# amorim-cleison/sign-language-nlp

Measured on AMD Instinct MI355X. Metric: train seq/s (batch=50,len=48), higher is better.
Workload: dtype bf16x3; 1 GPU; cfg2: Transformer train step E512 H8 N6 F512 batch 50 len 48 |src| 3000 |tgt| 202 dropout 0.1, fwd+CE+bwd+clip(0.5)+SGD(m=.9); launch=eager stream launches (auto: timed both in 9 untimed pre-warmup steps + warmup), per_gpu=independent fit (grid shard)

## Files before the change

### include/slnlp.h

```cpp
#ifndef SLNLP_H
#define SLNLP_H

#include <stdint.h>

#ifdef __cplusplus
extern "C" {
#endif

#define SLNLP_OK 0
#define SLNLP_ERR_INVALID_ARG 1
#define SLNLP_ERR_LAUNCH 2
#define SLNLP_ERR_UNSUPPORTED 3

#define SLNLP_ABI_VERSION 1

const char* slnlp_last_error(void);
int slnlp_abi_version(void);

typedef struct slnlp_gemm_args {
    const float* A; int64_t lda; int32_t a_kmajor;
    const float* B; int64_t ldb; int32_t b_kmajor;
    float* C; int64_t ldc;
    int32_t M, N, K;
    const float* bias;
    int32_t relu;
    const float* gate; int64_t ldg; float gate_scale;
    float drop_p; int32_t drop_site; const unsigned long long* rng;
    const float* resid; int64_t ldr;
    float* rowsum_a;
    int32_t precision;
    int32_t gate_mode;
    const uint16_t* A_hi; const uint16_t* A_lo; int64_t lda_p;
    const uint16_t* B_hi; const uint16_t* B_lo; int64_t ldb_p;
    uint16_t* C_hi; uint16_t* C_lo; int64_t ldc_p;
    int32_t drop_head_dim;
    const float* col_scale;
    uint8_t* C_q8;
    int32_t batch;
    int64_t batch_stride_a, batch_stride_b, batch_stride_c;
} slnlp_gemm_args;

int slnlp_gemm(const slnlp_gemm_args* args, void* stream);
int64_t slnlp_gemm_group_scratch_bytes(const slnlp_gemm_args* jobs, const int32_t* split_k, int njobs);
int slnlp_set_plane_tile(int tile);
int slnlp_set_gemm_ks(int ks);
int slnlp_set_rnn_step_tile(int rows16);
int slnlp_set_fp8_tile(int tile);
int slnlp_gemm_group(const slnlp_gemm_args* jobs, const int32_t* split_k, int njobs, void* scratch,
                     int64_t scratch_bytes, void* stream);
int slnlp_gemm_wd(const slnlp_gemm_args* wgrad, const slnlp_gemm_args* dgrad, void* scratch, int64_t scratch_bytes, void* stream);
int slnlp_gemm_wd_plan(const slnlp_gemm_args* wgrad, const slnlp_gemm_args* dgrad, int32_t* split, int32_t* separate, int32_t* geo_wgrad,
                       int32_t* geo_dgrad);
int slnlp_gemm_rows(const slnlp_gemm_args* args, void* stream);
int slnlp_gemm_rows_bwd(const slnlp_gemm_args* dgrad, const slnlp_gemm_args* wgrad, void* stream);
int slnlp_set_rows_tile(int tile);
int slnlp_quant_rows_fp8(const float* x, int64_t ld, int R, int K, uint8_t* q, int64_t ldq, float* scale, void* stream);
int slnlp_split_planes(const float* x, int64_t ld, int R, int C, uint16_t* hi, uint16_t* lo, int64_t ldp, void* stream);

int slnlp_embed_fwd(const int64_t* ids, int64_t ld_ids, int B, int S, int E, int V,
                    const float* table, const float* pe , float* out,
                    float scale ,
                    float drop_p, int drop_site, const unsigned long long* rng,
                    int64_t nan_idx , void* stream);
int64_t slnlp_embed_bwd_scratch_bytes(int B, int S, int E);
int slnlp_embed_bwd(const int64_t* ids, int64_t ld_ids, int B, int S, int E, int V,
                    const float* dx, float* dtable, float scale,
                    int64_t zero_row ,
                    float drop_p, int drop_site, const unsigned long long* rng,
                    void* scratch, void* stream);

int slnlp_attn_self_fwd(const float* qkv, const int64_t* ids, int64_t ld_ids, int64_t pad_idx,
                        int causal, int B, int S, int H, int dh,
                        float* ctx, float* probs,
                        float drop_p, int drop_site, const unsigned long long* rng, void* stream);
int slnlp_attn_self_bwd(const float* qkv, const float* probs, const float* dctx,
                        int B, int S, int H, int dh, float* dqkv,
                        float drop_p, int drop_site, const unsigned long long* rng, void* stream);

int64_t slnlp_attn_long_scratch_bytes(int B, int S, int H);
int slnlp_attn_self_bwd_long(const float* qkv, const float* probs, const float* dctx, int B, int S, int H, int dh,
                             float* dqkv, float* scratch, float drop_p, int drop_site, const unsigned long long* rng,
                             void* stream);
int slnlp_attn_cross_fwd(const float* q, const float* kv, int64_t ld_kv, int B, int S, int H, int dh,
                         float* ctx, float* probs,
                         float drop_p, int drop_site, const unsigned long long* rng, void* stream);
int slnlp_attn_cross_bwd(const float* q, const float* kv, int64_t ld_kv, const float* probs,
                         const float* dctx, int B, int S, int H, int dh,
                         float* dq, float* dkv, int64_t ld_dkv,
                         float drop_p, int drop_site, const unsigned long long* rng, void* stream);

int slnlp_layernorm_fwd(const float* x, const float* gamma, const float* beta, int rows, int E,
                        float eps, float* y, float* stats, void* stream);
#define SLNLP_LN_MAX_PARTIALS 1024
int slnlp_layernorm_bwd(const float* dy, const float* x, const float* gamma, const float* stats,
                        int rows, int E, const float* add_to_dx, float* dx, float* dx_drop,
                        float drop_p, int drop_site, const unsigned long long* rng,
                        float* partial, int* nblk_out, void* stream);
typedef struct slnlp_ln_reduce_entry {
    const float* partial; float* dgamma; float* dbeta; int32_t nblk; int32_t E;
} slnlp_ln_reduce_entry;
int slnlp_ln_param_reduce(const slnlp_ln_reduce_entry* table_dev, int n, int max_E, void* stream);

int slnlp_lsm_nll(const float* logits, int64_t ld_logits, const int64_t* y, int B, int V,
                  int64_t ignore_index, float* logp, float* loss, float* dlogits, int64_t ld_dlogits,
                  float* row_scratch , void* stream);
int slnlp_lsm_nll_ex(const float* logits, int64_t ld_logits, const int64_t* y, int B, int V, int64_t ignore_index,
                     const float* class_weight, float label_smoothing, int reduction, float* logp, float* loss,
                     float* dlogits, int64_t ld_dlogits, float* row_scratch , void* stream);
int slnlp_lsm_bwd(const float* logp, const float* dlogp, int B, int V, float* dlogits,
                  int64_t ld_dlogits, void* stream);

int slnlp_clip_sgd_step(float* params, const float* grads, float* momentum_buf, int64_t n,
                        const float* lr_dev, float momentum, float max_norm,
                        float* partials , float* norm_out,
                        unsigned long long* rng, void* stream);

int slnlp_clip_sgd_step_ex(float* params, const float* grads, float* momentum_buf, int64_t n, const float* lr_dev,
                           float momentum, float dampening, float weight_decay, int nesterov, float max_norm,
                           float* partials , float* norm_out, float* step_count, int64_t skip_begin,
                           int64_t skip_end, void* stream);
int slnlp_clip_adamw_step(float* params, const float* grads, float* exp_avg, float* exp_avg_sq, int64_t n,
                          const float* lr_dev, float beta1, float beta2, float eps, float weight_decay, float max_norm,
                          float* partials , float* norm_out, float* step_count, int64_t skip_begin,
                          int64_t skip_end, void* stream);

int slnlp_clip_adam_step(float* params, const float* grads, float* exp_avg, float* exp_avg_sq, int64_t n,
                         const float* lr_dev, float beta1, float beta2, float eps, float weight_decay, float max_norm,
                         float* partials , float* norm_out, float* step_count, void* stream);

int slnlp_dropout_mask(float* out, int R, int C, float p, int site,
                       const unsigned long long* rng, void* stream);

typedef struct slnlp_rnn_cell_dir {
    const float* xproj;
    const float* hproj;
    float* h;
    float* c;
    float* hprev_save;
    float* cprev_save;
    float* acts;
    float* hn_save;
    float* out;
    int32_t t, out_row0, out_col0;
} slnlp_rnn_cell_dir;
int slnlp_rnn_cell_fwd(int lstm, const slnlp_rnn_cell_dir* dirs, int ndir, int B, int Hd,
                       const int64_t* lengths, float fill, int64_t ld_out,
                       float drop_p, int drop_site, const unsigned long long* rng, void* stream);
typedef struct slnlp_rnn_step_dir {
    const float* h_in;
    float* h_out;
    const float* w_hh;
    const float* b_hh;
    const float* xproj;
    float* c;
    float* cprev_save;
    float* acts;
    float* hn_save;
    float* out;
    int32_t t, out_row0, out_col0;
} slnlp_rnn_step_dir;
int slnlp_rnn_step_fwd(int lstm, const slnlp_rnn_step_dir* dirs, int ndir, int B, int Hd,
                       const int64_t* lengths, float fill, int64_t ld_out,
                       float drop_p, int drop_site, const unsigned long long* rng, int precision, void* stream);
typedef struct slnlp_rnn_layer_dir {
    float* hprev;
    float* h_final;
    const float* w_hh;
    const float* b_hh;
    const float* xproj;
    float* c;
    float* cprev;
    float* acts;
    float* hn;
    float* out;
    int32_t out_col0;
    int32_t reverse;
} slnlp_rnn_layer_dir;
int slnlp_rnn_layer_fwd(int lstm, const slnlp_rnn_layer_dir* dirs, int ndir, int B, int Hd, int S,
                        const int64_t* lengths, float fill, int64_t ld_out,
                        float drop_p, int drop_site, const unsigned long long* rng, int precision,
                        uint32_t* sync, int* launched, void* stream);
typedef struct slnlp_rnn_cell_bwd_dir {
    float* dh_state; float* dc_state;
    const float* dout;
    const float* acts; const float* cprev_save; const float* hprev_save; const float* hn_save;
    float* dgx; float* dgh; float* carry;
    int32_t t, out_row0, out_col0;
    const float* dh_extra; int64_t extra_stride; int32_t n_extra;
} slnlp_rnn_cell_bwd_dir;
int slnlp_rnn_cell_bwd(int lstm, const slnlp_rnn_cell_bwd_dir* dirs, int ndir, int B, int Hd,
                       const int64_t* lengths, int64_t ld_dout,
                       float drop_p, int drop_site, const unsigned long long* rng, void* stream);

typedef struct slnlp_rnn_step_bwd_dir {
    slnlp_rnn_cell_bwd_dir cell;
    const float* dgh_next;
    const float* w_hh;
} slnlp_rnn_step_bwd_dir;
int slnlp_rnn_step_bwd(int lstm, const slnlp_rnn_step_bwd_dir* dirs, int ndir, int B, int Hd,
                       const int64_t* lengths, int64_t ld_dout,
                       float drop_p, int drop_site, const unsigned long long* rng, int precision, void* stream);

int slnlp_bahdanau_fwd(const float* q, const float* proj_key, const float* value, const float* w_energy,
                       const int64_t* ids, int64_t ld_ids, int64_t pad_idx, int B, int S, int Hd,
                       float* alphas, float* ctx, void* stream);
int slnlp_bahdanau_bwd(const float* q, const float* proj_key, const float* value, const float* w_energy,
// ... 142 lines not shown
```

### sign-language-nlp_amd/csrc/common.hpp

```cpp
#pragma once
#include <vector>
#include <hip/hip_runtime.h>
#include <atomic>
#include <mutex>
#include <stdint.h>
#include <stdio.h>
#include <string.h>

#include "../../include/slnlp.h"

namespace slnlp {

void set_error(const char* fmt, ...);

#define SLNLP_CHECK_ARG(cond, ...)                 \
    do {                                           \
        if (!(cond)) {                             \
            ::slnlp::set_error(__VA_ARGS__);       \
            return SLNLP_ERR_INVALID_ARG;          \
        }                                          \
    } while (0)

#define SLNLP_CHECK_LAUNCH(what)                                              \
    do {                                                                      \
// ... 24 lines not shown
        std::lock_guard<std::mutex> lk(mu);
        if (done[dev].load(std::memory_order_relaxed)) return 0;
        const int rc = init();
        if (rc == 0) done[dev].store(true, std::memory_order_release);
        return rc;
    }
};

#ifndef SLNLP_PROBE_FENCES
#define SLNLP_PROBE_FENCES 0
#endif
__device__ __forceinline__ void probe_kernel_begin() {
#if SLNLP_PROBE_FENCES & 1
    __builtin_amdgcn_fence(__ATOMIC_ACQUIRE, "agent");
    asm volatile("s_waitcnt vmcnt(0)" ::: "memory");
#endif
}
__device__ __forceinline__ void probe_kernel_end() {
#if SLNLP_PROBE_FENCES & 2
    asm volatile("s_waitcnt vmcnt(0)" ::: "memory");
    __builtin_amdgcn_fence(__ATOMIC_RELEASE, "agent");
    asm volatile("s_waitcnt vmcnt(0)" ::: "memory");
#endif
}

struct RngState {
    unsigned long long seed;
    unsigned long long step;
};

struct DropKey { unsigned ks[5]; };
__device__ __forceinline__ DropKey dropout_key(const unsigned long long* rng, int site) {
    const unsigned long long k = rng[0] + 0x9E3779B97F4A7C15ull * rng[1];
    DropKey K;
    K.ks[0] = (unsigned)k; K.ks[1] = (unsigned)(k >> 32); K.ks[2] = (unsigned)site; K.ks[3] = 0u;
    K.ks[4] = 0x1BD11BDAu ^ K.ks[0] ^ K.ks[1] ^ K.ks[2] ^ K.ks[3];
    return K;
}

#ifndef SLNLP_THREEFRY_ROUNDS
#define SLNLP_THREEFRY_ROUNDS 12
#endif
__device__ __forceinline__ uint4 threefry4x32(unsigned c0, unsigned c1, const DropKey& K) {
    constexpr int ROT[8][2] = {{10, 26}, {11, 21}, {13, 27}, {23, 5}, {6, 20}, {17, 11}, {25, 10}, {18, 20}};
    unsigned x0 = c0 + K.ks[0], x1 = c1 + K.ks[1], x2 = K.ks[2], x3 = K.ks[3];
#pragma unroll
    for (int r = 0; r < SLNLP_THREEFRY_ROUNDS; ++r) {
        if ((r & 1) == 0) {
            x0 += x1; x1 = __builtin_rotateleft32(x1, ROT[r & 7][0]) ^ x0;
            x2 += x3; x3 = __builtin_rotateleft32(x3, ROT[r & 7][1]) ^ x2;
        } else {
            x0 += x3; x3 = __builtin_rotateleft32(x3, ROT[r & 7][0]) ^ x0;
            x2 += x1; x1 = __builtin_rotateleft32(x1, ROT[r & 7][1]) ^ x2;
        }
        if ((r & 3) == 3) {
            const int s = (r + 1) >> 2;
            x0 += K.ks[s % 5]; x1 += K.ks[(s + 1) % 5]; x2 += K.ks[(s + 2) % 5]; x3 += K.ks[(s + 3) % 5] + (unsigned)s;
        }
    }
    return make_uint4(x0, x1, x2, x3);
}

__device__ __forceinline__ unsigned drop_cc(unsigned c) { return ((c >> 5) << 4) | (c & 15u); }
__device__ __forceinline__ int drop_half(unsigned c) { return (int)((c >> 4) & 1u); }

__device__ __forceinline__ uint4 dropout_bits8(const DropKey& key, unsigned r4, unsigned cc) { return threefry4x32(cc, r4, key); }

__host__ __device__ __forceinline__ unsigned dropout_threshold(float p) {
    const double t = (double)p * 65536.0 + 0.5;
    return t >= 65535.0 ? 65535u : (unsigned)t;
}

__device__ __forceinline__ unsigned pick_lot(const uint4& v, int half, int r) {
    const unsigned long long lo = (unsigned long long)v.x | ((unsigned long long)v.y << 32);
    const unsigned long long hi = (unsigned long long)v.z | ((unsigned long long)v.w << 32);
    return (unsigned)((half ? hi : lo) >> (16 * (r & 3))) & 0xFFFFu;
}

__device__ __forceinline__ bool dropout_keep(const DropKey& key, unsigned r, unsigned c, unsigned thr) {
    const uint4 b = dropout_bits8(key, r >> 2, drop_cc(c));
    return pick_lot(b, drop_half(c), (int)(r & 3u)) >= thr;
}
__device__ __forceinline__ bool dropout_keep(const unsigned long long* rng, int site,
                                             unsigned r, unsigned c, unsigned thr) {
    return dropout_keep(dropout_key(rng, site), r, c, thr);
}

struct PlaneOut {
    unsigned short* hi = nullptr;
    unsigned short* lo = nullptr;
    unsigned char* q8 = nullptr;
};
__device__ __forceinline__ unsigned pack_fp8x4(float a, float b, float c, float d) {
    a = fminf(fmaxf(a, -448.f), 448.f); b = fminf(fmaxf(b, -448.f), 448.f);
    c = fminf(fmaxf(c, -448.f), 448.f); d = fminf(fmaxf(d, -448.f), 448.f);
    int w = __builtin_amdgcn_cvt_pk_fp8_f32(a, b, 0, false);
    w = __builtin_amdgcn_cvt_pk_fp8_f32(c, d, w, true);
    return (unsigned)w;
}
__device__ __forceinline__ void split_bf16(float x, unsigned short& h, unsigned short& l) {
    const __bf16 hb = (__bf16)x;
    h = __builtin_bit_cast(unsigned short, hb);
    const __bf16 b = (__bf16)(x - (float)hb);
    l = __builtin_bit_cast(unsigned short, b);
}
__device__ __forceinline__ unsigned short head_bf16(float x) { return __builtin_bit_cast(unsigned short, (__bf16)x); }
__device__ __forceinline__ void store_planes1(const PlaneOut& po, long idx, float v) {
    if (!po.hi) return;
    unsigned short h, l;
    split_bf16(v, h, l);
    po.hi[idx] = h;
    po.lo[idx] = l;
    if (po.q8) po.q8[idx] = (unsigned char)(pack_fp8x4(v, 0.f, 0.f, 0.f) & 0xFFu);
}
__device__ __forceinline__ void store_planes4(const PlaneOut& po, long idx, float4 v) {
    if (!po.hi) return;
    unsigned short h[4], l[4];
    split_bf16(v.x, h[0], l[0]); split_bf16(v.y, h[1], l[1]); split_bf16(v.z, h[2], l[2]); split_bf16(v.w, h[3], l[3]);
    uint2 w;
    w.x = h[0] | ((unsigned)h[1] << 16); w.y = h[2] | ((unsigned)h[3] << 16);
    *reinterpret_cast<uint2*>(po.hi + idx) = w;
    w.x = l[0] | ((unsigned)l[1] << 16); w.y = l[2] | ((unsigned)l[3] << 16);
    *reinterpret_cast<uint2*>(po.lo + idx) = w;
    if (po.q8) *reinterpret_cast<unsigned*>(po.q8 + idx) = pack_fp8x4(v.x, v.y, v.z, v.w);
}

template <int CTRL>
__device__ __forceinline__ float dpp_mov(float v) {
    return __builtin_bit_cast(float, __builtin_amdgcn_update_dpp(0, __builtin_bit_cast(int, v), CTRL, 0xF, 0xF, true));
}
constexpr int DPP_XOR1 = 0xB1, DPP_XOR2 = 0x4E;
constexpr int DPP_HALF_MIRROR = 0x141, DPP_MIRROR = 0x140;
__device__ __forceinline__ float lane_bcast(float v, int lane) {
    return __builtin_bit_cast(float, __builtin_amdgcn_readlane(__builtin_bit_cast(int, v), lane));
}
__device__ __forceinline__ float row16_sum(float v) {
    v += dpp_mov<DPP_XOR1>(v);
    v += dpp_mov<DPP_XOR2>(v);
    v += dpp_mov<DPP_HALF_MIRROR>(v);
    v += dpp_mov<DPP_MIRROR>(v);
    return v;
}
__device__ __forceinline__ float row16_max(float v) {
    v = fmaxf(v, dpp_mov<DPP_XOR1>(v));
    v = fmaxf(v, dpp_mov<DPP_XOR2>(v));
    v = fmaxf(v, dpp_mov<DPP_HALF_MIRROR>(v));
    v = fmaxf(v, dpp_mov<DPP_MIRROR>(v));
    return v;
}
__device__ __forceinline__ float wave_sum(float v) {
    v = row16_sum(v);
    return (lane_bcast(v, 0) + lane_bcast(v, 16)) + (lane_bcast(v, 32) + lane_bcast(v, 48));
}
__device__ __forceinline__ float wave_max(float v) {
    v = row16_max(v);
    return fmaxf(fmaxf(lane_bcast(v, 0), lane_bcast(v, 16)), fmaxf(lane_bcast(v, 32), lane_bcast(v, 48)));
}

}

namespace slnlp {
int gemm(const slnlp_gemm_args& a, hipStream_t s);
int gemm_group(const slnlp_gemm_args* jobs, int njobs, hipStream_t s, unsigned wide_mask = 0);
int gemm_planes(const slnlp_gemm_args& a, hipStream_t s);
int gemm_rows(const slnlp_gemm_args& a, hipStream_t s);
int gemm_rows_bwd(const slnlp_gemm_args& dgrad, const slnlp_gemm_args& wgrad, hipStream_t s);
int gemm_planes_init();
int gemm_planes_group(const slnlp_gemm_args* jobs, const int* split_k, int njobs, void* scratch, size_t scratch_bytes,
                      hipStream_t s, bool defer_reduce = false);
size_t gemm_group_scratch_bytes(const slnlp_gemm_args* jobs, const int* split_k, int njobs);
constexpr int WD_MAX_SPLITK = 8;
struct WdPlan { int split, separate; };
WdPlan gemm_planes_wd_plan(const slnlp_gemm_args& wgrad, const slnlp_gemm_args& dgrad);
int gemm_planes_wd(const slnlp_gemm_args& wgrad, const slnlp_gemm_args& dgrad, void* scratch, size_t scratch_bytes, hipStream_t s);
struct QuantRow { long off; int K, pad; };
int quant_rows_fp8(const float* x, int64_t ld, int R, int K, unsigned char* q, int64_t ldq, float* scale, const void* row_table,
                   hipStream_t st);
int split_planes(const float* x, int64_t ld, int R, int C, unsigned short* hi, unsigned short* lo, int64_t ldp, hipStream_t st);
int embed_fwd(const int64_t* ids, int64_t ld_ids, int B, int S, int E, int V, const float* table, const float* pe,
              float* out, float scale, float drop_p, int drop_site, const unsigned long long* rng, int64_t nan_idx,
              hipStream_t st, PlaneOut po = {}, unsigned char* keep_mask = nullptr);
int embed_bwd(const int64_t* ids, int64_t ld_ids, int B, int S, int E, int V, const float* dx, float* dtable,
              float scale, int64_t zero_row, float drop_p, int drop_site, const unsigned long long* rng, void* scratch,
              hipStream_t st, const unsigned char* keep_mask = nullptr);
size_t embed_bwd_scratch_bytes(int B, int S, int E);
int attn_self_fwd(const float* qkv, const int64_t* ids, int64_t ld_ids, int64_t pad_idx, int causal, int B, int S,
                  int H, int dh, float* ctx, float* probs, float drop_p, int drop_site,
                  const unsigned long long* rng, hipStream_t st, PlaneOut po = {});
int attn_self_bwd(const float* qkv, const float* probs, const float* dctx, int B, int S, int H, int dh, float* dqkv,
                  float drop_p, int drop_site, const unsigned long long* rng, hipStream_t st, PlaneOut po = {},
                  float* long_scratch = nullptr);
size_t attn_long_scratch_bytes(int B, int S, int H);
int attn_cross_fwd(const float* q, const float* kv, int64_t ld_kv, int B, int S, int H, int dh, float* ctx,
                   float* probs, float drop_p, int drop_site, const unsigned long long* rng, hipStream_t st);
int attn_cross_bwd(const float* q, const float* kv, int64_t ld_kv, const float* probs, const float* dctx, int B,
                   int S, int H, int dh, float* dq, float* dkv, int64_t ld_dkv, float drop_p, int drop_site,
                   const unsigned long long* rng, hipStream_t st, PlaneOut po = {});
int xmem_fwd(const float* qk, const float* mem, const float* bv, int B, int S, int H, int dh, float* mbar, float* psum, float* probs,
             float* ctx0, float drop_p, int drop_site, const unsigned long long* rng, hipStream_t st);
int xmem_bwd(const float* mem, const float* bv, const float* probs, const float* psum, const float* qk, const float* dmbar,
             const float* dctx, int B, int S, int H, int dh, float* dsc, float* dqk, float* dcp, float* dbv, float* dmem, int accumulate,
             float drop_p, int drop_site, const unsigned long long* rng, hipStream_t st);
int layernorm_fwd(const float* x, const float* gamma, const float* beta, int rows, int E, float eps, float* y,
                  float* stats, hipStream_t st, PlaneOut po = {});
int ln_bwd_blocks(int rows);
bool ln_bwd_fused(int full_rows);
int layernorm_bwd(const float* dy, const float* x, const float* gamma, const float* stats, int rows, int E,
                  const float* add_to_dx, float* dx, float* dx_drop, float drop_p, int drop_site,
                  const unsigned long long* rng, float* partial, int* nblk_out, int full_rows, hipStream_t st,
                  PlaneOut po_dx = {}, PlaneOut po_drop = {});
int attn_init();
int ln_param_reduce(const slnlp_ln_reduce_entry* table_dev, int n, int max_E, hipStream_t st);
struct LnPartialEntry {
    const float* dy;
    const float* x;
    const float* stats;
    float* partial;
    int dec;
    int pad;
};
int ln_param_partial(const LnPartialEntry* table_dev, const LnPartialEntry* single_host, int n, int E, int rows_enc, int rows_dec,
                     int full_rows_enc, int full_rows_dec, hipStream_t st);
int ln_partial_chunk(int rows);
struct LossOpts {
    const float* class_weight = nullptr;
    float label_smoothing = 0.f;
    int reduction = 0;
};
int lsm_nll(const float* logits, int64_t ld_logits, const int64_t* y, int B, int V, int64_t ignore_index, float* logp,
            float* loss, float* dlogits, int64_t ld_dlogits, float* row_scratch, hipStream_t st, hipStream_t loss_st,
            float* logp2 = nullptr, const int* logp2_row = nullptr, float* loss_hist = nullptr, const int* hist_idx = nullptr,
            LossOpts lo = {});
int lsm_bwd(const float* logp, const float* dlogp, int B, int V, float* dlogits, int64_t ld_dlogits, hipStream_t st);
int rnn_cell_fwd(int lstm, const slnlp_rnn_cell_dir* dirs, int ndir, int B, int Hd, const int64_t* lengths, float fill,
                 int64_t ld_out, float drop_p, int drop_site, const unsigned long long* rng, hipStream_t st);
int rnn_step_fwd(int lstm, const slnlp_rnn_step_dir* dirs, int ndir, int B, int Hd, const int64_t* lengths, float fill,
                 int64_t ld_out, float drop_p, int drop_site, const unsigned long long* rng, int precision, hipStream_t st);
int rnn_layer_init();
int rnn_layer_fwd(int lstm, const slnlp_rnn_layer_dir* dirs, int ndir, int B, int Hd, int S, const int64_t* lengths,
                  float fill, int64_t ld_out, float drop_p, int drop_site, const unsigned long long* rng, int precision,
                  unsigned* bar, int* err, int* launched, hipStream_t st);
int rnn_cell_bwd(int lstm, const slnlp_rnn_cell_bwd_dir* dirs, int ndir, int B, int Hd, const int64_t* lengths,
                 int64_t ld_dout, float drop_p, int drop_site, const unsigned long long* rng, hipStream_t st);
bool rnn_step_bwd_covers(int B, int Hd);
int rnn_step_bwd_init();
int rnn_step_bwd(int lstm, const slnlp_rnn_step_bwd_dir* dirs, int ndir, int B, int Hd, const int64_t* lengths, int64_t ld_dout,
                 float drop_p, int drop_site, const unsigned long long* rng, int precision, hipStream_t st);
int bahdanau_fwd(const float* q, const float* pk, const float* val, const float* we, const int64_t* ids,
                 int64_t ld_ids, int64_t pad, int B, int S, int Hd, float* alphas, float* ctx, hipStream_t st);
int bahdanau_bwd(const float* q, const float* pk, const float* val, const float* we, const float* alphas,
                 const float* dctx, int B, int S, int Hd, float* dq, float* dpk, float* dval, float* dwe_part,
                 float* dwe, hipStream_t st);
int add_rows(const float* in, int64_t ld_in, float* out, int64_t ld_out, int R, int C, int accumulate, hipStream_t st);
int tanh_bwd(const float* dy, const float* y, float* out, int64_t n, hipStream_t st);
struct SgdOpts {
    float dampening = 0.f, weight_decay = 0.f;
    int nesterov = 0;
    float* steps = nullptr;
    int64_t skip_begin = 0, skip_end = 0;
};
struct AdamOpts {
    int decoupled = 0;
    int64_t skip_begin = 0, skip_end = 0;
};
int clip_sgd_step(float* params, const float* grads, float* momentum_buf, int64_t n, const float* lr_dev,
                  float momentum, float max_norm, float* partials, float* norm_out, unsigned long long* rng,
                  hipStream_t st, PlaneOut wp = {}, int64_t wp_begin = 0, int64_t wp_end = -1,
                  SgdOpts so = {});
int clip_adam_step(float* params, const float* grads, float* exp_avg, float* exp_avg_sq, int64_t n, const float* lr_dev,
                   float beta1, float beta2, float eps, float weight_decay, float max_norm, float* partials, float* norm_out,
                   unsigned long long* rng, float* step_f, hipStream_t st, PlaneOut wp = {}, int64_t wp_begin = 0, int64_t wp_end = -1,
                   AdamOpts ao = {});
struct TrainOpts {
    float* class_weight = nullptr;
    std::vector<float> class_weight_host;
    float label_smoothing = 0.f;
    int reduction = 0;
    int kind = 0;
    float dampening = 0.f, weight_decay = 0.f;
    int nesterov = 0;
    unsigned gen = 0;
    TrainOpts() = default;
    TrainOpts(const TrainOpts&) = delete;
    TrainOpts& operator=(const TrainOpts&) = delete;
    ~TrainOpts();
    LossOpts loss() const { return LossOpts{class_weight, label_smoothing, reduction}; }
    SgdOpts sgd(float* steps, int64_t skip_begin, int64_t skip_end) const {
        if (kind != 0) return SgdOpts{0.f, 0.f, 0, steps, skip_begin, skip_end};
        return SgdOpts{dampening, weight_decay, nesterov, steps, skip_begin, skip_end};
    }
    AdamOpts adam(int64_t skip_begin, int64_t skip_end) const { return AdamOpts{kind == 2 ? 1 : 0, skip_begin, skip_end}; }
    float adam_weight_decay(float group) const { return kind == 0 ? group : weight_decay; }
    int set_criterion(int V, const float* cw, float eps, int reduction, hipStream_t st, bool* changed);
    int set_update(int kind, float dampening, float weight_decay, int nesterov, bool* changed);
};

unsigned long long params_generation(const float* params);
unsigned long long bump_params_generation(const float* params);
}
```

### sign-language-nlp_amd/csrc/elementwise.hip

```cpp
#include "common.hpp"
#include "launch.hpp"

namespace slnlp {

__device__ __forceinline__ void embed_fwd_body(const long* __restrict__ ids, long ld_ids, int B, int S,
                                                        int E, int V, const float* __restrict__ table,
                                                        const float* __restrict__ pe, float* __restrict__ out,
                                                        float scale, float drop_p, unsigned drop_thr, int drop_site,
                                                        const unsigned long long* __restrict__ rng, long nan_idx,
                                                        PlaneOut po, unsigned char* __restrict__ keep_mask) {
    const int e4 = E >> 2;
    const long total = (long)B * S * e4;
    const float ik = 1.f / (1.f - drop_p);
    for (long idx = blockIdx.x * 256L + threadIdx.x; idx < total; idx += (long)gridDim.x * 256) {
        const int m = (int)(idx / e4), c = (int)(idx % e4) * 4;
        const int s = m / B, b = m % B;
        const long id = ids[(long)b * ld_ids + s];
        float4 v = make_float4(0.f, 0.f, 0.f, 0.f);
        if (id >= 0 && id < V) v = *reinterpret_cast<const float4*>(table + id * E + c);
        const float4 p = pe ? *reinterpret_cast<const float4*>(pe + (long)s * E + c) : make_float4(0.f, 0.f, 0.f, 0.f);
        v.x = v.x * scale + p.x; v.y = v.y * scale + p.y; v.z = v.z * scale + p.z; v.w = v.w * scale + p.w;
        if (drop_p > 0.f) {
            const bool k0 = dropout_keep(rng, drop_site, m, c + 0, drop_thr), k1 = dropout_keep(rng, drop_site, m, c + 1, drop_thr);
            const bool k2 = dropout_keep(rng, drop_site, m, c + 2, drop_thr), k3 = dropout_keep(rng, drop_site, m, c + 3, drop_thr);
// ... 108 lines not shown
        if ((tid & 63) == 0) match[tid >> 6] = bal;
        __syncthreads();
        if (tid == 0) {
            int n = nlist;
            for (int w = 0; w < 4; ++w) {
                unsigned long long bits = match[w];
                while (bits && n < 1024) {
                    list[n++] = base + w * 64 + __ffsll((long long)bits) - 1;
                    bits &= bits - 1;
                }
            }
            nlist = n;
        }
        __syncthreads();
    }
    const int n = nlist;
    __shared__ __attribute__((aligned(16))) float red[4][256];
    const int wave = tid >> 6, lane = tid & 63, per = (n + 3) / 4;
    const int i0 = wave * per, i1 = (i0 + per < n) ? i0 + per : n;
    for (int c0 = 0; c0 < E; c0 += 256) {
        const int c = c0 + lane * 4;
        float4 acc = make_float4(0.f, 0.f, 0.f, 0.f);
        if (c < E) {
            for (int i = i0; i < i1; i += 4) {
                float4 g[4];
#pragma unroll
                for (int u = 0; u < 4; ++u)
                    g[u] = (i + u < i1) ? *reinterpret_cast<const float4*>(partial + (long)list[i + u] * E + c)
                                        : make_float4(0.f, 0.f, 0.f, 0.f);
#pragma unroll
                for (int u = 0; u < 4; ++u) { acc.x += g[u].x; acc.y += g[u].y; acc.z += g[u].z; acc.w += g[u].w; }
            }
        }
        if (c0 > 0) __syncthreads();
        *reinterpret_cast<float4*>(&red[wave][lane * 4]) = acc;
        __syncthreads();
        if (wave == 0 && c < E) {
            float4 r = *reinterpret_cast<const float4*>(&red[0][lane * 4]);
#pragma unroll
            for (int w = 1; w < 4; ++w) {
                const float4 q = *reinterpret_cast<const float4*>(&red[w][lane * 4]);
                r.x += q.x; r.y += q.y; r.z += q.z; r.w += q.w;
            }
            r.x *= scale; r.y *= scale; r.z *= scale; r.w *= scale;
            *reinterpret_cast<float4*>(dtable + (long)id * E + c) = r;
        }
    }
}
SLNLP_ZKERNEL(embed_bwd_combine_kernel, 256, embed_bwd_combine_body)

__device__ __forceinline__ void embed_bwd_small_body(const long* __restrict__ ids, long ld_ids, int B, int S, int E, int V,
                                                     const float* __restrict__ dx, float* __restrict__ dtable, float scale,
                                                     float drop_p, unsigned drop_thr, int drop_site,
                                                     const unsigned long long* __restrict__ rng) {
    const int M = B * S, lane = threadIdx.x & 63, m = blockIdx.x;
    int my_id = -1;
    if (lane < M) {
        const long v = ids[(long)(lane % B) * ld_ids + (lane / B)];
        my_id = (v < 0 || v >= V) ? -1 : (int)v;
    }
    if (m < V && __ballot(my_id == m) == 0ull) {
        for (int c = threadIdx.x * 4; c < E; c += 1024) *reinterpret_cast<float4*>(dtable + (long)m * E + c) = make_float4(0.f, 0.f, 0.f, 0.f);
    }
    if (m >= M) return;
    const float ik = 1.f / (1.f - drop_p);
    const int id = __builtin_amdgcn_readlane(my_id, __builtin_amdgcn_readfirstlane(m));
    const unsigned long long mask = __ballot(my_id == id && id >= 0);
    const bool first = id >= 0 && (mask & ((1ull << m) - 1ull)) == 0ull;
    if (!first) return;
    __shared__ __attribute__((aligned(16))) float red[4][256];
    const int wave = threadIdx.x >> 6;
    const unsigned long long wmask = mask & (0xFFFFull << (16 * wave));
    for (int c0 = 0; c0 < E; c0 += 256) {
        const int c = c0 + lane * 4;
        float4 acc = make_float4(0.f, 0.f, 0.f, 0.f);
        if (c < E) {
            unsigned long long bits = wmask;
            while (bits) {
                int k[4];
#pragma unroll
                for (int u = 0; u < 4; ++u) {
                    k[u] = bits ? __ffsll((long long)bits) - 1 : -1;
                    bits &= bits - 1;
                }
                float4 g[4];
#pragma unroll
                for (int u = 0; u < 4; ++u)
                    g[u] = k[u] >= 0 ? load_dx_row(dx, k[u], E, c, drop_p, ik, drop_thr, drop_site, rng, nullptr)
                                     : make_float4(0.f, 0.f, 0.f, 0.f);
#pragma unroll
                for (int u = 0; u < 4; ++u) { acc.x += g[u].x; acc.y += g[u].y; acc.z += g[u].z; acc.w += g[u].w; }
            }
        }
        if (c0 > 0) __syncthreads();
        *reinterpret_cast<float4*>(&red[wave][lane * 4]) = acc;
        __syncthreads();
        if (wave == 0 && c < E) {
            float4 r = *reinterpret_cast<const float4*>(&red[0][lane * 4]);
#pragma unroll
            for (int w = 1; w < 4; ++w) {
                const float4 q = *reinterpret_cast<const float4*>(&red[w][lane * 4]);
                r.x += q.x; r.y += q.y; r.z += q.z; r.w += q.w;
            }
            r.x *= scale; r.y *= scale; r.z *= scale; r.w *= scale;
            *reinterpret_cast<float4*>(dtable + (long)id * E + c) = r;
        }
    }
}
SLNLP_ZKERNEL(embed_bwd_small_kernel, 256, embed_bwd_small_body)

int embed_fwd(const int64_t* ids, int64_t ld_ids, int B, int S, int E, int V, const float* table, const float* pe,
              float* out, float scale, float drop_p, int drop_site, const unsigned long long* rng, int64_t nan_idx,
              hipStream_t st, PlaneOut po, unsigned char* keep_mask) {
    SLNLP_CHECK_ARG(ids && table && out, "embed_fwd: null pointer");
    SLNLP_CHECK_ARG(B > 0 && S > 0 && V > 0 && E > 0 && E % 4 == 0, "embed_fwd: bad shape B=%d S=%d E=%d V=%d", B, S, E, V);
    SLNLP_CHECK_ARG(drop_p >= 0.f && drop_p < 1.f && (drop_p == 0.f || rng), "embed_fwd: bad dropout args");
    const long total = (long)B * S * (E / 4);
    int grid = ceil_div(total, 256);
    if (grid > 2048) grid = 2048;
    SLNLP_TRY(zlaunch(embed_fwd_kernel, dim3(grid), 256, 0, st, "embed_fwd",
                      (const long*)ids, (long)ld_ids, B, S, E, V, table, pe, out, scale, drop_p, dropout_threshold(drop_p), drop_site, rng, (long)nan_idx, po, keep_mask));
    return 0;
}

size_t embed_bwd_scratch_bytes(int B, int S, int E) {
    return ((size_t)B * S * E * sizeof(float) + (size_t)B * S * sizeof(int) + 255) & ~(size_t)255;
}

int embed_bwd(const int64_t* ids, int64_t ld_ids, int B, int S, int E, int V, const float* dx, float* dtable,
              float scale, int64_t zero_row, float drop_p, int drop_site, const unsigned long long* rng, void* scratch,
              hipStream_t st, const unsigned char* keep_mask) {
    SLNLP_CHECK_ARG(ids && dx && dtable && scratch, "embed_bwd: null pointer");
    SLNLP_CHECK_ARG(B > 0 && S > 0 && V > 0 && E > 0 && E % 4 == 0, "embed_bwd: bad shape");
    SLNLP_CHECK_ARG((long)B * S <= 65536, "embed_bwd: more than 65536 tokens per batch");
    SLNLP_CHECK_ARG(drop_p >= 0.f && drop_p < 1.f && (drop_p == 0.f || rng), "embed_bwd: bad dropout args");
    const int M = B * S;
    if (M <= EMB_CHUNK && !keep_mask) {
        SLNLP_TRY(zlaunch(embed_bwd_small_kernel, dim3(M > V ? M : V), 256, 0, st, "embed_bwd_small",
                          (const long*)ids, (long)ld_ids, B, S, E, V, dx, dtable, scale, drop_p, dropout_threshold(drop_p), drop_site, rng));
        if (zero_row >= 0 && zero_row < V) SLNLP_TRY(fill_zero(dtable + zero_row * E, (size_t)E * sizeof(float), st));
        return 0;
    }
    SLNLP_TRY(fill_zero(dtable, (size_t)V * E * sizeof(float), st));
    float* partial = (float*)scratch;
    int* pid = (int*)(partial + (size_t)M * E);
    SLNLP_TRY(zlaunch(embed_bwd_chunk_kernel, dim3(M), 256, 0, st, "embed_bwd_chunk",
                      (const long*)ids, (long)ld_ids, B, S, E, V, dx, partial, pid, drop_p, dropout_threshold(drop_p), drop_site, rng, keep_mask));
    SLNLP_TRY(zlaunch(embed_bwd_combine_kernel, dim3(M), 256, 0, st, "embed_bwd_combine",
                      pid, M, E, partial, dtable, scale));
    if (zero_row >= 0 && zero_row < V) SLNLP_TRY(fill_zero(dtable + zero_row * E, (size_t)E * sizeof(float), st));
    return 0;
}

constexpr int LN_MAXU = 4;

__device__ __forceinline__ void layernorm_fwd_body(const float* __restrict__ x,
                                                            const float* __restrict__ gamma,
                                                            const float* __restrict__ beta, int rows, int E,
                                                            float eps, float* __restrict__ y,
                                                            float* __restrict__ stats, PlaneOut po) {
    const int lane = threadIdx.x & 63, wave = threadIdx.x >> 6;
    const int row = blockIdx.x * 4 + wave;
    if (row >= rows) return;
    const float* xr = x + (long)row * E;
    float4 v[LN_MAXU], g[LN_MAXU], bt[LN_MAXU];
#pragma unroll
    for (int u = 0; u < LN_MAXU; ++u) {
        const int c = lane * 4 + u * 256;
        const bool in = c < E;
        v[u] = in ? *reinterpret_cast<const float4*>(xr + c) : make_float4(0.f, 0.f, 0.f, 0.f);
        g[u] = in ? *reinterpret_cast<const float4*>(gamma + c) : make_float4(0.f, 0.f, 0.f, 0.f);
        bt[u] = in ? *reinterpret_cast<const float4*>(beta + c) : make_float4(0.f, 0.f, 0.f, 0.f);
    }
    float s = 0.f;
#pragma unroll
    for (int u = 0; u < LN_MAXU; ++u) s += v[u].x + v[u].y + v[u].z + v[u].w;
    const float mean = wave_sum(s) / (float)E;
    float q = 0.f;
#pragma unroll
    for (int u = 0; u < LN_MAXU; ++u) {
        if (lane * 4 + u * 256 < E) {
            const float a = v[u].x - mean, b = v[u].y - mean, cc = v[u].z - mean, d = v[u].w - mean;
            q += a * a + b * b + cc * cc + d * d;
        }
    }
    const float rstd = 1.f / sqrtf(wave_sum(q) / (float)E + eps);
#pragma unroll
    for (int u = 0; u < LN_MAXU; ++u) {
        const int c = lane * 4 + u * 256;
        if (c < E) {
            float4 o;
            o.x = (v[u].x - mean) * rstd * g[u].x + bt[u].x; o.y = (v[u].y - mean) * rstd * g[u].y + bt[u].y;
            o.z = (v[u].z - mean) * rstd * g[u].z + bt[u].z; o.w = (v[u].w - mean) * rstd * g[u].w + bt[u].w;
            *reinterpret_cast<float4*>(y + (long)row * E + c) = o;
            store_planes4(po, (long)row * E + c, o);
        }
    }
    if (lane == 0 && stats) {
        stats[2 * row] = mean;
        stats[2 * row + 1] = rstd;
    }
}
SLNLP_ZKERNEL(layernorm_fwd_kernel, 256, layernorm_fwd_body)

template <int U, int GS, int RB, bool FUSE>
__device__ __forceinline__ void layernorm_bwd_rows(
    const float* __restrict__ dy, const float* __restrict__ x, const float* __restrict__ gamma,
    const float* __restrict__ stats, int rows, int E, const float* __restrict__ add_to_dx, float* __restrict__ dx,
    float* __restrict__ dx_drop, float drop_p, unsigned drop_thr, int drop_site,
    const unsigned long long* __restrict__ rng, PlaneOut po_dx, PlaneOut po_drop, float* __restrict__ partial, int chunk_rows, int nchunks) {
    const int lane = threadIdx.x & 63, wave = threadIdx.x >> 6;
    const float invE = 1.f / (float)E, ik = 1.f / (1.f - drop_p);
    const bool want_drop = dx_drop != nullptr || po_drop.hi != nullptr;
    const bool drop = want_drop && drop_p > 0.f;
    const int unit = FUSE ? (int)blockIdx.x : blockIdx.x * (int)(blockDim.x >> 6) + wave;
    float4 ag[U], ab[U];
#pragma unroll
    for (int u = 0; u < U; ++u) ag[u] = ab[u] = make_float4(0.f, 0.f, 0.f, 0.f);
    const int row_begin = FUSE ? unit * chunk_rows + wave * GS : unit * GS;
    const int row_end = FUSE ? ((unit + 1) * chunk_rows < rows ? (unit + 1) * chunk_rows : rows) : row_begin + GS;
    const int row_step = FUSE ? 4 * GS : GS;
    if (!FUSE && row_begin >= rows) return;
    DropKey dkey = {};
    if (drop) dkey = dropout_key(rng, drop_site);
    float4 g[U];
#pragma unroll
    for (int u = 0; u < U; ++u)
        if (lane * 4 + u * 256 < E) g[u] = *reinterpret_cast<const float4*>(gamma + lane * 4 + u * 256);
#pragma unroll 1
    for (int row0 = row_begin; row0 < row_end; row0 += row_step)
#pragma unroll
    for (int i0 = 0; i0 < GS; i0 += RB) {
        float4 d[RB][U], v[RB][U];
        float mean[RB], rstd[RB], s1[RB], s2[RB];
#pragma unroll
        for (int i = 0; i < RB; ++i) {
            const int row = row0 + i0 + i < rows ? row0 + i0 + i : rows - 1;
            mean[i] = stats[2 * row];
            rstd[i] = stats[2 * row + 1];
#pragma unroll
            for (int u = 0; u < U; ++u) {
                const int c = lane * 4 + u * 256;
                if (c < E) {
                    d[i][u] = *reinterpret_cast<const float4*>(dy + (long)row * E + c);
                    v[i][u] = *reinterpret_cast<const float4*>(x + (long)row * E + c);
                }
            }
        }
#pragma unroll
        for (int i = 0; i < RB; ++i) {
            float a1 = 0.f, a2 = 0.f;
#pragma unroll
            for (int u = 0; u < U; ++u) {
                if (lane * 4 + u * 256 < E) {
                    const float4 dd = d[i][u], vv = v[i][u];
                    const float4 xh = make_float4((vv.x - mean[i]) * rstd[i], (vv.y - mean[i]) * rstd[i], (vv.z - mean[i]) * rstd[i], (vv.w - mean[i]) * rstd[i]);
                    const float4 gv = make_float4(dd.x * g[u].x, dd.y * g[u].y, dd.z * g[u].z, dd.w * g[u].w);
                    a1 += gv.x + gv.y + gv.z + gv.w;
                    a2 += gv.x * xh.x + gv.y * xh.y + gv.z * xh.z + gv.w * xh.w;
                }
            }
            s1[i] = wave_sum(a1) * invE;
            s2[i] = wave_sum(a2) * invE;
        }
#pragma unroll
        for (int u = 0; u < U; ++u) {
            const int c = lane * 4 + u * 256;
            if (c >= E) continue;
            uint4 kb[4];
            const int half = drop_half((unsigned)c);
            if (drop) {
#pragma unroll
                for (int e = 0; e < 4; ++e) kb[e] = dropout_bits8(dkey, (unsigned)(row0 + i0) >> 2, drop_cc((unsigned)(c + e)));
            }
#pragma unroll
            for (int i = 0; i < RB; ++i) {
                const int row = row0 + i0 + i;
                if (row >= rows) continue;
                const int wsel = row & 3;
                const float4 dd = d[i][u], vv = v[i][u];
                const float4 xh = make_float4((vv.x - mean[i]) * rstd[i], (vv.y - mean[i]) * rstd[i], (vv.z - mean[i]) * rstd[i], (vv.w - mean[i]) * rstd[i]);
                const float4 gv = make_float4(dd.x * g[u].x, dd.y * g[u].y, dd.z * g[u].z, dd.w * g[u].w);
                if (FUSE) {
                    ag[u].x += dd.x * xh.x; ag[u].y += dd.y * xh.y; ag[u].z += dd.z * xh.z; ag[u].w += dd.w * xh.w;
                    ab[u].x += dd.x; ab[u].y += dd.y; ab[u].z += dd.z; ab[u].w += dd.w;
                }
                float4 o;
                o.x = rstd[i] * (gv.x - s1[i] - xh.x * s2[i]); o.y = rstd[i] * (gv.y - s1[i] - xh.y * s2[i]);
                o.z = rstd[i] * (gv.z - s1[i] - xh.z * s2[i]); o.w = rstd[i] * (gv.w - s1[i] - xh.w * s2[i]);
                if (add_to_dx) {
                    const float4 a = *reinterpret_cast<const float4*>(add_to_dx + (long)row * E + c);
                    o.x += a.x; o.y += a.y; o.z += a.z; o.w += a.w;
                }
                *reinterpret_cast<float4*>(dx + (long)row * E + c) = o;
                store_planes4(po_dx, (long)row * E + c, o);
                if (want_drop) {
                    if (drop) {
                        o.x = pick_lot(kb[0], half, wsel) >= drop_thr ? o.x * ik : 0.f;
                        o.y = pick_lot(kb[1], half, wsel) >= drop_thr ? o.y * ik : 0.f;
                        o.z = pick_lot(kb[2], half, wsel) >= drop_thr ? o.z * ik : 0.f;
                        o.w = pick_lot(kb[3], half, wsel) >= drop_thr ? o.w * ik : 0.f;
                    }
                    if (dx_drop) *reinterpret_cast<float4*>(dx_drop + (long)row * E + c) = o;
                    store_planes4(po_drop, (long)row * E + c, o);
                }
            }
        }
    }
    if (FUSE) {
        __shared__ float4 red[4][2][U * 64];
#pragma unroll
        for (int u = 0; u < U; ++u) {
            red[wave][0][u * 64 + lane] = ag[u];
            red[wave][1][u * 64 + lane] = ab[u];
        }
        __syncthreads();
        for (int q = threadIdx.x; q < 2 * U * 64; q += 256) {
            const int which = q / (U * 64), slot = q - which * (U * 64), c = (slot & 63) * 4 + (slot >> 6) * 256;
            if (c >= E) continue;
            float4 t = red[0][which][slot];
#pragma unroll
            for (int k = 1; k < 4; ++k) {
                const float4 o = red[k][which][slot];
                t.x += o.x; t.y += o.y; t.z += o.z; t.w += o.w;
            }
            *reinterpret_cast<float4*>(partial + ((long)unit * 2 + which) * E + c) = t;
        }
    }
}

#define SLNLP_LN_BWD_BODY(name, U, GS, RB, FUSE)                                                                                    \
    __device__ __forceinline__ void name(const float* __restrict__ dy, const float* __restrict__ x, const float* __restrict__ gamma, \
                                         const float* __restrict__ stats, int rows, int E, const float* __restrict__ add_to_dx,     \
                                         float* __restrict__ dx, float* __restrict__ dx_drop, float drop_p, unsigned drop_thr,       \
                                         int drop_site, const unsigned long long* __restrict__ rng, PlaneOut po_dx,                  \
                                         PlaneOut po_drop, float* __restrict__ partial, int chunk_rows, int nchunks) {               \
        layernorm_bwd_rows<U, GS, RB, FUSE>(dy, x, gamma, stats, rows, E, add_to_dx, dx, dx_drop, drop_p, drop_thr, drop_site, rng, \
                                            po_dx, po_drop, partial, chunk_rows, nchunks);                                          \
    }
SLNLP_LN_BWD_BODY(layernorm_bwd_body_u1g4, 1, 4, 4, false)
SLNLP_LN_BWD_BODY(layernorm_bwd_body_u2g4, 2, 4, 4, false)
SLNLP_LN_BWD_BODY(layernorm_bwd_body_u4g4, 4, 4, 2, false)
SLNLP_LN_BWD_BODY(layernorm_bwd_body_u1g1, 1, 1, 1, false)
SLNLP_LN_BWD_BODY(layernorm_bwd_body_u2g1, 2, 1, 1, false)
SLNLP_LN_BWD_BODY(layernorm_bwd_body_u4g1, 4, 1, 1, false)
SLNLP_LN_BWD_BODY(layernorm_bwd_body_u1g4f, 1, 4, 4, true)
SLNLP_LN_BWD_BODY(layernorm_bwd_body_u2g4f, 2, 4, 4, true)
SLNLP_LN_BWD_BODY(layernorm_bwd_body_u4g4f, 4, 4, 2, true)
// ... 662 lines not shown
```

### sign-language-nlp_amd/csrc/gemm_rows.hip

```cpp
#include <algorithm>
#include <atomic>

#include "common.hpp"
#include "gemm_jobs.hpp"
#include "launch.hpp"

namespace slnlp {

typedef __attribute__((ext_vector_type(8))) __bf16 bf16x8;
typedef __attribute__((ext_vector_type(4))) float f32x4;

struct RowsParams {
    slnlp_gemm_args a;
    unsigned drop_thr;
    float drop_scale;
};
__device__ __forceinline__ RowsParams as_global(RowsParams p) {
    launder(p.a);
    return p;
}

#if SLNLP_PROBE_FENCES == 256
constexpr int RTS_MAX = 1 << 14, RTS_W = 6;
__device__ unsigned long long g_rts[RTS_MAX][RTS_W];
__device__ unsigned g_rts_n;
#define RTS_MARK(slot) do { if (threadIdx.x == 0) rts[slot] = __builtin_amdgcn_s_memrealtime(); } while (0)
#else
#define RTS_MARK(slot) do { } while (0)
#endif

constexpr int RT_THREADS = 512, RT_WAVES = 8;
constexpr int RT_MAX_KTILES = 16;

typedef __attribute__((ext_vector_type(4))) short s16x4;
typedef __attribute__((ext_vector_type(8))) short s16x8;
typedef __attribute__((address_space(3))) void* lds_vp;
typedef __attribute__((address_space(1))) const void* glb_vp;

constexpr int RT_IMG = 64 * 16;
__device__ __forceinline__ void rows_dma_image(const unsigned short* __restrict__ plane, long ld, int k0, int r0, unsigned short* img, int lane) {
#pragma unroll
    for (int q = 0; q < 2; ++q) {
        const unsigned short* src = plane + (long)(k0 + 32 * q + (lane >> 1)) * ld + r0 + 8 * (lane & 1);
        __builtin_amdgcn_global_load_lds((glb_vp)src, (lds_vp)(img + q * 512), 16, 0, 0);
    }
}
__device__ __forceinline__ bf16x8 rows_tr_frag(const unsigned short* img, int kk, int lane) {
    const int i = lane & 15, kb = kk * 32 + ((lane >> 4) << 3) + (i >> 2);
    const unsigned short* p0 = img + kb * 16 + ((i & 3) << 2);
    typedef __attribute__((address_space(3))) s16x4* lds_p;
    const s16x4 v0 = __builtin_amdgcn_ds_read_tr16_b64_v4i16((lds_p)(p0));
    const s16x4 v1 = __builtin_amdgcn_ds_read_tr16_b64_v4i16((lds_p)(p0 + 4 * 16));
    const s16x8 v = {v0[0], v0[1], v0[2], v0[3], v1[0], v1[1], v1[2], v1[3]};
    return __builtin_bit_cast(bf16x8, v);
}

template <int NSPLIT>
__device__ __forceinline__ void rows_split8(const float (&x)[8], bf16x8& hi, bf16x8& lo) {
#pragma unroll
    for (int e = 0; e < 8; ++e) {
        const __bf16 h = (__bf16)x[e];
        hi[e] = h;
        if (NSPLIT == 3) lo[e] = (__bf16)(x[e] - (float)h);
    }
}
__device__ __forceinline__ void rows_load8(const float* __restrict__ p, float (&x)[8]) {
    const float4 a = *reinterpret_cast<const float4*>(p), b = *reinterpret_cast<const float4*>(p + 4);
    x[0] = a.x; x[1] = a.y; x[2] = a.z; x[3] = a.w; x[4] = b.x; x[5] = b.y; x[6] = b.z; x[7] = b.w;
}
constexpr int RT_FIMG = 64 * 16;
__device__ __forceinline__ void rows_dma_image_f32(const float* __restrict__ W, long ld, int k0, int c0, int N, float* img, int lane) {
#pragma unroll
    for (int q = 0; q < 4; ++q) {
        const int c = min(c0 + 4 * (lane & 3), N - 4);
        const float* src = W + (long)(k0 + 16 * q + (lane >> 2)) * ld + c;
        __builtin_amdgcn_global_load_lds((glb_vp)src, (lds_vp)(img + q * 256), 16, 0, 0);
    }
}
__device__ __forceinline__ void rows_img_col8(const float* img, int kk, int lane, float (&x)[8]) {
    const float* p = img + (kk * 32 + ((lane >> 4) << 3)) * 16 + (lane & 15);
#pragma unroll
    for (int e = 0; e < 8; ++e) x[e] = p[e * 16];
}

template <int NSPLIT, int MT, int NT, bool BK>
__device__ __forceinline__ void rows_tile(const RowsParams& p, int bx, int by, float* part) {
    static_assert(MT * NT <= RT_WAVES, "one epilogue tile per wave");
    const slnlp_gemm_args& g = p.a;
    const int tid = threadIdx.x, lane = tid & 63, wave = __builtin_amdgcn_readfirstlane(tid >> 6);
#if SLNLP_PROBE_FENCES == 256
    unsigned long long rts[RTS_W] = {0, 0, 0, 0, 0, 0};
    struct RtsFlush {
        unsigned long long* t;
        __device__ ~RtsFlush() {
            if (threadIdx.x == 0) {
                t[4] = __builtin_amdgcn_s_memrealtime();
                t[5] = ((unsigned long long)(gridDim.x * gridDim.y) << 32) | (unsigned)(blockIdx.y * gridDim.x + blockIdx.x);
                const unsigned i = atomicAdd(&g_rts_n, 1u) & (unsigned)(RTS_MAX - 1);
                for (int k = 0; k < RTS_W; ++k) g_rts[i][k] = t[k];
            }
        }
    } rts_flush{rts};
    RTS_MARK(0);
#endif
    const int bn0 = bx * 16 * NT, bm0 = by * 16 * MT;
    const int M = g.M, N = g.N;
    const int ktiles = (g.K + 63) >> 6;
    const int am_last = ((M + 15) / 16 - 1) * 16, bn_last = ((N + 15) / 16 - 1) * 16;
    const long koct = 8 * (lane >> 4);
    const unsigned short *ah[MT], *al[MT];
    const float* bw[NT];
    int bcol[NT];
#pragma unroll
    for (int i = 0; i < MT; ++i) {
        const long off = (long)(min(bm0 + 16 * i, am_last) + (lane & 15)) * g.lda_p + koct;
        ah[i] = g.A_hi + off; al[i] = g.A_lo + off;
    }
#pragma unroll
    for (int j = 0; j < NT; ++j) {
        bcol[j] = min(bn0 + 16 * j, bn_last);
        bw[j] = g.B + (long)min(bcol[j] + (lane & 15), N - 1) * g.ldb + koct;
    }
    float* bimg = part + (size_t)ktiles * MT * NT * 256 + wave * NT * RT_FIMG;

    const int ei = wave / NT, ej = wave % NT;
    const int gm0 = bm0 + 16 * ei + ((lane >> 4) << 2), gn = bn0 + 16 * ej + (lane & 15);
    const bool live = wave < MT * NT && gn < N && gm0 < M;
    float bias = 0.f, gt[4] = {0.f, 0.f, 0.f, 0.f}, rs[4] = {0.f, 0.f, 0.f, 0.f};
    DropKey dkey = {};
    auto epilogue_loads = [&]() {
        if (!live) return;
        if (g.bias) bias = g.bias[gn];
#pragma unroll
        for (int r = 0; r < 4; ++r) {
            const int gm = gm0 + r < M ? gm0 + r : gm0;
            if (g.gate) gt[r] = g.gate[(long)gm * g.ldg + gn];
            if (g.resid) rs[r] = g.resid[(long)gm * g.ldr + gn];
        }
        if (g.drop_p > 0.f) dkey = dropout_key(g.rng, g.drop_site);
    };

    for (int t = wave; t < ktiles; t += RT_WAVES) {
        bf16x8 fa[2][MT], la[2][MT], fb[2][NT], lb[2][NT];
        if (!BK) {
            if (t != wave) asm volatile("s_waitcnt lgkmcnt(0)" ::: "memory");
#pragma unroll
            for (int j = 0; j < NT; ++j) rows_dma_image_f32(g.B, g.ldb, t * 64, bcol[j], N, bimg + j * RT_FIMG, lane);
        }
#pragma unroll
        for (int kk = 0; kk < 2; ++kk) {
            const int k = t * 64 + kk * 32;
            if (BK) {
#pragma unroll
                for (int j = 0; j < NT; ++j) {
                    float x[8];
                    rows_load8(bw[j] + k, x);
                    rows_split8<NSPLIT>(x, fb[kk][j], lb[kk][j]);
                }
            }
#pragma unroll
            for (int i = 0; i < MT; ++i) {
                fa[kk][i] = *reinterpret_cast<const bf16x8*>(ah[i] + k);
                if (NSPLIT == 3) la[kk][i] = *reinterpret_cast<const bf16x8*>(al[i] + k);
            }
        }
        if (t == wave) epilogue_loads();
        if (!BK) {
            asm volatile("s_waitcnt vmcnt(0)" ::: "memory");
#pragma unroll
            for (int kk = 0; kk < 2; ++kk)
#pragma unroll
                for (int j = 0; j < NT; ++j) {
                    float x[8];
                    rows_img_col8(bimg + j * RT_FIMG, kk, lane, x);
                    rows_split8<NSPLIT>(x, fb[kk][j], lb[kk][j]);
                }
        }
#if SLNLP_PROBE_FENCES == 256
        if (t == 0) { asm volatile("s_waitcnt vmcnt(0)" ::: "memory"); RTS_MARK(1); }
#endif
        f32x4 acc[MT][NT];
#pragma unroll
        for (int i = 0; i < MT; ++i)
#pragma unroll
            for (int j = 0; j < NT; ++j) acc[i][j] = f32x4{0.f, 0.f, 0.f, 0.f};
#pragma unroll
        for (int kk = 0; kk < 2; ++kk)
#pragma unroll
            for (int i = 0; i < MT; ++i)
#pragma unroll
                for (int j = 0; j < NT; ++j) {
                    if (NSPLIT == 3) {
                        acc[i][j] = __builtin_amdgcn_mfma_f32_16x16x32_bf16(la[kk][i], fb[kk][j], acc[i][j], 0, 0, 0);
                        acc[i][j] = __builtin_amdgcn_mfma_f32_16x16x32_bf16(fa[kk][i], lb[kk][j], acc[i][j], 0, 0, 0);
                    }
                    acc[i][j] = __builtin_amdgcn_mfma_f32_16x16x32_bf16(fa[kk][i], fb[kk][j], acc[i][j], 0, 0, 0);
                }
#pragma unroll
        for (int i = 0; i < MT; ++i)
#pragma unroll
            for (int j = 0; j < NT; ++j) *reinterpret_cast<f32x4*>(part + (((t * MT + i) * NT + j) * 64 + lane) * 4) = acc[i][j];
    }
    if (wave >= ktiles) epilogue_loads();
    RTS_MARK(2);
    __syncthreads();
    if (wave >= MT * NT) return;
    f32x4 acc = *reinterpret_cast<const f32x4*>(part + (wave * 64 + lane) * 4);
    for (int t = 1; t < ktiles; ++t) acc += *reinterpret_cast<const f32x4*>(part + ((t * MT * NT + wave) * 64 + lane) * 4);
    RTS_MARK(3);
    if (!live) return;

    unsigned lot[4] = {0u, 0u, 0u, 0u};
    if (g.drop_p > 0.f) {
        if (g.drop_head_dim == 0) {
            const uint4 bits = dropout_bits8(dkey, (unsigned)gm0 >> 2, drop_cc((unsigned)gn));
            const int h = drop_half((unsigned)gn);
#pragma unroll
            for (int r = 0; r < 4; ++r) lot[r] = pick_lot(bits, h, r);
        } else {
#pragma unroll
            for (int r = 0; r < 4; ++r) {
                const unsigned rh = (unsigned)(gm0 + r) * (unsigned)(N / g.drop_head_dim) + (unsigned)(gn / g.drop_head_dim);
                lot[r] = pick_lot(dropout_bits8(dkey, rh >> 2, 0u), 0, (int)(rh & 3u));
            }
        }
    }
#pragma unroll
    for (int r = 0; r < 4; ++r) {
        const int gm = gm0 + r;
        if (gm >= M) break;
        float v = acc[r] + bias;
        if (g.relu == 1) v = fmaxf(v, 0.f);
        else if (g.relu == 2) v = tanhf(v);
        if (g.gate) v = g.gate_mode == 1 ? v * (1.f - gt[r] * gt[r]) : (gt[r] > 0.f ? v * g.gate_scale : 0.f);
        if (g.drop_p > 0.f) v = (lot[r] >= p.drop_thr) ? v * p.drop_scale : 0.f;
        if (g.resid) v += rs[r];
        if (g.C) g.C[(long)gm * g.ldc + gn] = v;
        if (g.C_hi) {
            unsigned short h, l;
            split_bf16(v, h, l);
            g.C_hi[(long)gm * g.ldc_p + gn] = h;
            if (g.C_lo) g.C_lo[(long)gm * g.ldc_p + gn] = l;
        }
    }
}

template <int NSPLIT, int WM>
__device__ __forceinline__ void rows_wgrad_unit(const slnlp_gemm_args& g, int unit, unsigned short* smem) {
    constexpr int NP = NSPLIT == 3 ? 2 : 1;
    const int tid = threadIdx.x, lane = tid & 63, wave = __builtin_amdgcn_readfirstlane(tid >> 6);
    const int M = g.M, N = g.N, ktiles = (g.K + 63) >> 6;
    const int units_n = (N + 127) / 128, um = unit / units_n, un = unit - um * units_n;
    const int m0 = um * 16 * WM, n0 = un * 128 + wave * 16, m_last = ((M + 15) / 16 - 1) * 16;
    const bool active = n0 < N;
    unsigned short* aimg = smem;
    unsigned short* bimg = smem + WM * 2 * RT_IMG + wave * 2 * RT_IMG;
    f32x4 total[WM], rsum[WM];
#pragma unroll
    for (int i = 0; i < WM; ++i) { total[i] = f32x4{0.f, 0.f, 0.f, 0.f}; rsum[i] = f32x4{0.f, 0.f, 0.f, 0.f}; }
    const bool do_rs = g.rowsum_a != nullptr && un == 0 && wave == 0;
    bf16x8 ones;
#pragma unroll
    for (int e = 0; e < 8; ++e) ones[e] = (__bf16)1.0f;
#if SLNLP_PROBE_FENCES == 256
    unsigned long long rts[RTS_W] = {0, 0, 0, 0, 0, 0};
    struct RtsFlushW {
        unsigned long long* t;
        unsigned tag;
        __device__ ~RtsFlushW() {
            if (threadIdx.x == 0) {
                t[4] = __builtin_amdgcn_s_memrealtime();
                t[5] = ((unsigned long long)(gridDim.x * gridDim.y) << 32) | tag | (unsigned)(blockIdx.y * gridDim.x + blockIdx.x);
                const unsigned i = atomicAdd(&g_rts_n, 1u) & (unsigned)(RTS_MAX - 1);
                for (int k = 0; k < RTS_W; ++k) g_rts[i][k] = t[k];
            }
        }
    } rts_flush{rts, 0x80000000u | (g.rowsum_a != nullptr && un == 0 ? 0x40000000u : 0u)};
    RTS_MARK(0);
#endif
    for (int t = 0; t < ktiles; ++t) {
        if (t) {
            asm volatile("s_waitcnt lgkmcnt(0)" ::: "memory");
            __syncthreads();
        }
        for (int im = wave; im < WM * NP; im += RT_WAVES) {
            const int i = im / NP, pl = im - i * NP;
            rows_dma_image(pl ? g.A_lo : g.A_hi, g.lda_p, t * 64, min(m0 + 16 * i, m_last), aimg + (2 * i + pl) * RT_IMG, lane);
        }
        if (active) {
            rows_dma_image(g.B_hi, g.ldb_p, t * 64, n0, bimg, lane);
            if (NSPLIT == 3) rows_dma_image(g.B_lo, g.ldb_p, t * 64, n0, bimg + RT_IMG, lane);
        }
        asm volatile("s_waitcnt vmcnt(0)" ::: "memory");
        __syncthreads();
#if SLNLP_PROBE_FENCES == 256
        if (t == 0) RTS_MARK(1);
#endif
        if (active) {
            bf16x8 fb[2], lb[2];
#pragma unroll
            for (int kk = 0; kk < 2; ++kk) {
                fb[kk] = rows_tr_frag(bimg, kk, lane);
                if (NSPLIT == 3) lb[kk] = rows_tr_frag(bimg + RT_IMG, kk, lane);
            }
#pragma unroll
            for (int i = 0; i < WM; ++i) {
                f32x4 acc = f32x4{0.f, 0.f, 0.f, 0.f}, rs = f32x4{0.f, 0.f, 0.f, 0.f};
#pragma unroll
                for (int kk = 0; kk < 2; ++kk) {
                    const bf16x8 fa = rows_tr_frag(aimg + (2 * i) * RT_IMG, kk, lane);
                    if (NSPLIT == 3) {
                        const bf16x8 la = rows_tr_frag(aimg + (2 * i + 1) * RT_IMG, kk, lane);
                        acc = __builtin_amdgcn_mfma_f32_16x16x32_bf16(la, fb[kk], acc, 0, 0, 0);
                        acc = __builtin_amdgcn_mfma_f32_16x16x32_bf16(fa, lb[kk], acc, 0, 0, 0);
                        if (do_rs) rs = __builtin_amdgcn_mfma_f32_16x16x32_bf16(la, ones, rs, 0, 0, 0);
                    }
                    acc = __builtin_amdgcn_mfma_f32_16x16x32_bf16(fa, fb[kk], acc, 0, 0, 0);
                    if (do_rs) rs = __builtin_amdgcn_mfma_f32_16x16x32_bf16(fa, ones, rs, 0, 0, 0);
                }
                total[i] = t == 0 ? acc : total[i] + acc;
                if (do_rs) rsum[i] = t == 0 ? rs : rsum[i] + rs;
            }
        }
#if SLNLP_PROBE_FENCES == 256
        if (t == 0) RTS_MARK(2);
#endif
    }
    RTS_MARK(3);
    if (!active) return;
    const int gn = n0 + (lane & 15);
#pragma unroll
    for (int i = 0; i < WM; ++i) {
        const int gm0 = m0 + 16 * i + ((lane >> 4) << 2);
        if (gn < N) {
#pragma unroll
            for (int r = 0; r < 4; ++r)
                if (gm0 + r < M) g.C[(long)(gm0 + r) * g.ldc + gn] = total[i][r];
        }
        if (do_rs && (lane & 15) == 0) {
#pragma unroll
            for (int r = 0; r < 4; ++r)
                if (gm0 + r < M) g.rowsum_a[gm0 + r] = rsum[i][r];
        }
    }
}

template <int NSPLIT, int MT, int NT>
__device__ __forceinline__ void gemm_rows_body(RowsParams p) {
    extern __shared__ __attribute__((aligned(16))) float part[];
    rows_tile<NSPLIT, MT, NT, true>(p, blockIdx.x, blockIdx.y, part);
}

struct RowsBwdParams {
    RowsParams d;
    slnlp_gemm_args w;
};
__device__ __forceinline__ RowsBwdParams as_global(RowsBwdParams p) {
    launder(p.d.a);
    launder(p.w);
    return p;
}
template <int NSPLIT, int MT, int NT>
__device__ __forceinline__ void gemm_rows_bwd_body(RowsBwdParams p) {
    extern __shared__ __attribute__((aligned(16))) float part[];
    const int gx = (p.d.a.N + 16 * NT - 1) / (16 * NT), gy = (p.d.a.M + 16 * MT - 1) / (16 * MT), nd = gx * gy;
    const int id = blockIdx.x;
    if (id < nd) rows_tile<NSPLIT, MT, NT, false>(p.d, id % gx, id / gx, part);
    else rows_wgrad_unit<NSPLIT, MT>(p.w, id - nd, reinterpret_cast<unsigned short*>(part));
}

struct RowsGeo { int mt, nt; };
constexpr int RT_NGEO = 3;
constexpr RowsGeo RT_GEO[RT_NGEO] = {{1, 1}, {4, 1}, {4, 2}};
#define SLNLP_ROWS_KERNEL(NS, G)                                                                                          \
    __device__ __forceinline__ void gemm_rows_body_##NS##_##G(RowsParams p) { gemm_rows_body<NS, RT_GEO[G].mt, RT_GEO[G].nt>(p); } \
    SLNLP_ZKERNEL(gemm_rows_kernel_##NS##_##G, RT_THREADS, gemm_rows_body_##NS##_##G)                                     \
    __device__ __forceinline__ void gemm_rows_bwd_body_##NS##_##G(RowsBwdParams p) { gemm_rows_bwd_body<NS, RT_GEO[G].mt, RT_GEO[G].nt>(p); } \
    SLNLP_ZKERNEL(gemm_rows_bwd_kernel_##NS##_##G, RT_THREADS, gemm_rows_bwd_body_##NS##_##G)
SLNLP_ROWS_KERNEL(3, 0)
SLNLP_ROWS_KERNEL(3, 1)
SLNLP_ROWS_KERNEL(3, 2)
SLNLP_ROWS_KERNEL(1, 0)
SLNLP_ROWS_KERNEL(1, 1)
SLNLP_ROWS_KERNEL(1, 2)

using RowsKernel = void (*)(Pack<RowsParams>, const Pack<RowsParams>*);
using RowsBwdKernel = void (*)(Pack<RowsBwdParams>, const Pack<RowsBwdParams>*);
static RowsKernel rows_kernel(int precision, int geo) {
    if (precision == 3) return geo == 0 ? gemm_rows_kernel_3_0 : geo == 1 ? gemm_rows_kernel_3_1 : gemm_rows_kernel_3_2;
    return geo == 0 ? gemm_rows_kernel_1_0 : geo == 1 ? gemm_rows_kernel_1_1 : gemm_rows_kernel_1_2;
}
static RowsBwdKernel rows_bwd_kernel(int precision, int geo) {
    if (precision == 3) return geo == 0 ? gemm_rows_bwd_kernel_3_0 : geo == 1 ? gemm_rows_bwd_kernel_3_1 : gemm_rows_bwd_kernel_3_2;
    return geo == 0 ? gemm_rows_bwd_kernel_1_0 : geo == 1 ? gemm_rows_bwd_kernel_1_1 : gemm_rows_bwd_kernel_1_2;
}
static size_t rows_lds(int geo, int K) { return (size_t)ceil_div(K, 64) * RT_GEO[geo].mt * RT_GEO[geo].nt * 64 * 4 * sizeof(float); }
static size_t rows_bwd_lds(int geo, int K) {
    const size_t d = rows_lds(geo, K) + (size_t)RT_WAVES * RT_GEO[geo].nt * RT_FIMG * sizeof(float);
    const size_t w = (size_t)(RT_GEO[geo].mt + RT_WAVES) * 2 * RT_IMG * sizeof(unsigned short);
    return d > w ? d : w;
}
static dim3 rows_grid(int geo, int M, int N) { return dim3(ceil_div(N, 16 * RT_GEO[geo].nt), ceil_div(M, 16 * RT_GEO[geo].mt)); }
static int rows_wgrad_units(const slnlp_gemm_args& w, int geo) { return ceil_div(w.M, 16 * RT_GEO[geo].mt) * ceil_div(w.N, 128); }

static std::atomic<int> g_rows_geo{[] { const char* e = getenv("SLNLP_ROWS_TILE"); const int v = e ? atoi(e) : -1; return v >= 0 && v < RT_NGEO ? v : -1; }()};
constexpr size_t RT_LDS_MAX = 160 * 1024;
static int rows_geo(int M, int N, int K, int fits, bool bwd) {
    const int forced = g_rows_geo.load(std::memory_order_relaxed);
    auto fits_lds = [&](int geo) { return (bwd ? rows_bwd_lds(geo, K) : rows_lds(geo, K)) <= RT_LDS_MAX; };
    if (forced >= 0 && fits_lds(forced)) return forced;
    int best = 0;
    long best_cost = -1;
    for (int geo = 0; geo < RT_NGEO; ++geo) {
        if (!fits_lds(geo)) continue;
        const dim3 gr = rows_grid(geo, M, N);
        const long wunits = bwd ? (long)ceil_div(K, 16 * RT_GEO[geo].mt) * ceil_div(N, 128) : 0;
        const long units = ((long)gr.x * gr.y + wunits) * fits, rounds = (units + 255) / 256;
        const long cost = rounds * (16L * (RT_GEO[geo].mt + RT_GEO[geo].nt) * K * 4 + 16384);
        if (best_cost < 0 || cost < best_cost) { best_cost = cost; best = geo; }
    }
    return best;
}

static int rows_init() {
    static DeviceOnce once;
    return once.run([]() -> int {
        bool ok = true;
        for (int prec = 1; prec <= 3; prec += 2)
            for (int geo = 0; geo < RT_NGEO; ++geo)
                ok = ok && hipFuncSetAttribute((const void*)rows_kernel(prec, geo), hipFuncAttributeMaxDynamicSharedMemorySize,
                                               (int)std::min(rows_lds(geo, 64 * RT_MAX_KTILES), RT_LDS_MAX)) == hipSuccess &&
                     hipFuncSetAttribute((const void*)rows_bwd_kernel(prec, geo), hipFuncAttributeMaxDynamicSharedMemorySize,
                                         (int)std::min(rows_bwd_lds(geo, 64 * RT_MAX_KTILES), RT_LDS_MAX)) == hipSuccess;
        if (!ok) {
            set_error("gemm_rows: cannot raise dynamic LDS limit: %s", hipGetErrorString(hipGetLastError()));
            return SLNLP_ERR_LAUNCH;
        }
        return 0;
    });
}

const void* gemm_rows_for_fits(const void* fn, const void* recorded_args, int fits, dim3* grid, size_t* lds) {
    int prec = 0;
    bool bwd = false;
    for (int geo = 0; geo < RT_NGEO; ++geo) {
        if (fn == (const void*)rows_kernel(3, geo)) prec = 3;
        if (fn == (const void*)rows_kernel(1, geo)) prec = 1;
        if (fn == (const void*)rows_bwd_kernel(3, geo)) { prec = 3; bwd = true; }
        if (fn == (const void*)rows_bwd_kernel(1, geo)) { prec = 1; bwd = true; }
    }
    if (!prec) return nullptr;
    if (bwd) {
        const RowsBwdParams& P = *reinterpret_cast<const RowsBwdParams*>(recorded_args);
        const int geo = rows_geo(P.d.a.M, P.d.a.N, P.d.a.K, fits, true);
        const dim3 gr = rows_grid(geo, P.d.a.M, P.d.a.N);
        *grid = dim3(gr.x * gr.y + rows_wgrad_units(P.w, geo));
        *lds = rows_bwd_lds(geo, P.d.a.K);
        return (const void*)rows_bwd_kernel(prec, geo);
    }
    const slnlp_gemm_args& a = reinterpret_cast<const RowsParams*>(recorded_args)->a;
    const int geo = rows_geo(a.M, a.N, a.K, fits, false);
    *grid = rows_grid(geo, a.M, a.N);
    *lds = rows_lds(geo, a.K);
    return (const void*)rows_kernel(prec, geo);
}

static int check_rows_job(const slnlp_gemm_args& a, bool b_kmajor, const char* who) {
    SLNLP_CHECK_ARG(a.A_hi && a.B, "%s: A as bf16 planes (A_hi / A_lo / lda_p) and the weight B as fp32 (B / ldb) required", who);
    SLNLP_CHECK_ARG(a.a_kmajor && (a.b_kmajor != 0) == b_kmajor, "%s: operand layouts (A k-major; B k-major for a forward product, m-major for a data gradient)", who);
    SLNLP_CHECK_ARG(a.C || a.C_hi, "%s: no output", who);
    SLNLP_CHECK_ARG(a.M > 0 && a.N > 0 && a.K > 0, "%s: bad shape M=%d N=%d K=%d", who, a.M, a.N, a.K);
    SLNLP_CHECK_ARG(a.precision == 1 || (a.precision == 3 && a.A_lo), "%s: precision 1, or 3 with A's lo plane", who);
    SLNLP_CHECK_ARG(a.lda_p % 64 == 0 && a.lda_p >= a.K, "%s: A's plane row stride must be a multiple of 64 and cover K (zero-padded)", who);
    SLNLP_CHECK_ARG(a.K % 64 == 0 && a.ldb % 4 == 0 && a.ldb >= (b_kmajor ? a.K : a.N) && (b_kmajor || a.N % 4 == 0),
                    "%s: K must be a multiple of 64 (the fp32 weight has no padding), ldb a multiple of 4 that covers a row", who);
    SLNLP_CHECK_ARG((((uintptr_t)a.A_hi | (uintptr_t)a.A_lo | (uintptr_t)a.B) & 15) == 0, "%s: operands must be 16-byte aligned", who);
    SLNLP_CHECK_ARG(!a.C || a.ldc >= a.N, "%s: ldc < N", who);
    SLNLP_CHECK_ARG(!a.C_hi || a.ldc_p >= a.N, "%s: ldc_p < N", who);
    SLNLP_CHECK_ARG(a.drop_p >= 0.f && a.drop_p < 1.f && (a.drop_p == 0.f || a.rng), "%s: bad dropout args", who);
    SLNLP_CHECK_ARG(!a.gate || a.ldg >= a.N, "%s: ldg too small", who);
    SLNLP_CHECK_ARG(!a.resid || a.ldr >= a.N, "%s: ldr too small", who);
    SLNLP_CHECK_ARG(!a.rowsum_a && a.batch <= 1, "%s: no row sums, no batched jobs", who);
    SLNLP_CHECK_ARG(a.drop_head_dim >= 0 && (a.drop_head_dim == 0 || a.N % a.drop_head_dim == 0), "%s: drop_head_dim %d does not divide N %d", who,
                    a.drop_head_dim, a.N);
    SLNLP_CHECK_ARG(ceil_div(a.K, 64) <= RT_MAX_KTILES, "%s: K = %d > %d (the workgroup's partial tiles live in LDS)", who, a.K, 64 * RT_MAX_KTILES);
    return 0;
}

int gemm_rows_bwd(const slnlp_gemm_args& dgrad, const slnlp_gemm_args& wgrad, hipStream_t st) {
    SLNLP_TRY(check_rows_job(dgrad, false, "gemm_rows_bwd (dgrad)"));
    const slnlp_gemm_args& w = wgrad;
    SLNLP_CHECK_ARG(w.A_hi && w.B_hi && w.C && !w.a_kmajor && !w.b_kmajor, "gemm_rows_bwd (wgrad): m-major operand planes and an fp32 output required");
    SLNLP_CHECK_ARG(w.precision == dgrad.precision && (w.precision == 1 || (w.A_lo && w.B_lo)), "gemm_rows_bwd (wgrad): same precision as the dgrad, lo planes for 3");
    SLNLP_CHECK_ARG(w.M > 0 && w.N > 0 && w.K > 0 && w.lda_p % 64 == 0 && w.ldb_p % 64 == 0 && w.lda_p >= w.M && w.ldb_p >= w.N && w.ldc >= w.N,
                    "gemm_rows_bwd (wgrad): bad shape / strides");
    SLNLP_CHECK_ARG((((uintptr_t)w.A_hi | (uintptr_t)w.B_hi | (uintptr_t)w.A_lo | (uintptr_t)w.B_lo) & 15) == 0, "gemm_rows_bwd (wgrad): planes must be 16-byte aligned");
    SLNLP_CHECK_ARG(!w.bias && !w.gate && !w.resid && w.drop_p == 0.f && !w.C_hi && w.relu == 0 && w.batch <= 1, "gemm_rows_bwd (wgrad): no epilogue");
    RowsBwdParams p;
    p.d.a = dgrad;
    p.d.drop_thr = dropout_threshold(dgrad.drop_p);
    p.d.drop_scale = 1.f / (1.f - dgrad.drop_p);
    p.w = wgrad;
    SLNLP_TRY(rows_init());
    const int geo = rows_geo(dgrad.M, dgrad.N, dgrad.K, 1, true);
    const dim3 gr = rows_grid(geo, dgrad.M, dgrad.N);
    return zlaunch(rows_bwd_kernel(dgrad.precision, geo), dim3(gr.x * gr.y + rows_wgrad_units(wgrad, geo)), RT_THREADS, rows_bwd_lds(geo, dgrad.K), st,
                   "gemm_rows_bwd", p);
}

int gemm_rows(const slnlp_gemm_args& a, hipStream_t st) {
    SLNLP_TRY(check_rows_job(a, true, "gemm_rows"));
    RowsParams p;
    p.a = a;
    p.drop_thr = dropout_threshold(a.drop_p);
    p.drop_scale = 1.f / (1.f - a.drop_p);
    SLNLP_TRY(rows_init());
    const int geo = rows_geo(a.M, a.N, a.K, 1, false);
    return zlaunch(rows_kernel(a.precision, geo), rows_grid(geo, a.M, a.N), RT_THREADS, rows_lds(geo, a.K), st, "gemm_rows", p);
}

}

#if SLNLP_PROBE_FENCES == 256
extern "C" int slnlp_probe_rows_ts(unsigned long long* dst, int max_entries) {
    unsigned n = 0;
    if (hipDeviceSynchronize() != hipSuccess) return -1;
    if (hipMemcpyFromSymbol(&n, HIP_SYMBOL(slnlp::g_rts_n), sizeof(n)) != hipSuccess) return -1;
    if (n > (unsigned)slnlp::RTS_MAX) n = slnlp::RTS_MAX;
    if ((int)n > max_entries) n = max_entries;
    if (n && hipMemcpyFromSymbol(dst, HIP_SYMBOL(slnlp::g_rts), (size_t)n * slnlp::RTS_W * sizeof(unsigned long long)) != hipSuccess) return -1;
    const unsigned zero = 0;
    if (hipMemcpyToSymbol(HIP_SYMBOL(slnlp::g_rts_n), &zero, sizeof(zero)) != hipSuccess) return -1;
    return (int)n;
}
#endif

extern "C" int slnlp_gemm_rows_bwd(const slnlp_gemm_args* dgrad, const slnlp_gemm_args* wgrad, void* stream) {
    if (!dgrad || !wgrad) {
        slnlp::set_error("gemm_rows_bwd: null args");
        return SLNLP_ERR_INVALID_ARG;
    }
    return slnlp::gemm_rows_bwd(*dgrad, *wgrad, (hipStream_t)stream);
}

extern "C" int slnlp_set_rows_tile(int tile) {
    if (tile < -1 || tile >= slnlp::RT_NGEO) {
        slnlp::set_error("set_rows_tile: %d (-1 = automatic, 0 = 16 x 16, 1 = 64 x 16, 2 = 64 x 32 outputs per workgroup)", tile);
        return SLNLP_ERR_INVALID_ARG;
    }
    slnlp::g_rows_geo.store(tile, std::memory_order_relaxed);
    return 0;
}

extern "C" int slnlp_gemm_rows(const slnlp_gemm_args* args, void* stream) {
    if (!args) {
        slnlp::set_error("gemm_rows: null args");
        return SLNLP_ERR_INVALID_ARG;
    }
    return slnlp::gemm_rows(*args, (hipStream_t)stream);
}
```

### sign-language-nlp_amd/csrc/tf_plan.hip

```cpp
#include <map>
#include <string>
#include <vector>

#include "common.hpp"
#include "launch.hpp"
#include "tf_plan.hpp"

using namespace slnlp;

extern "C" {

int slnlp_tf_num_params(const slnlp_tf_config* cfg) {
    if (check_cfg(cfg)) return -1;
    return (int)build_layout(*cfg).ents.size();
}

int slnlp_tf_param_info(const slnlp_tf_config* cfg, int i, char* name, int64_t shape[2], int* ndim, int64_t* offset) {
    SLNLP_TRY(check_cfg(cfg));
    Layout L = build_layout(*cfg);
    SLNLP_CHECK_ARG(i >= 0 && i < (int)L.ents.size(), "tf_param_info: index %d out of range", i);
    const ParamEnt& e = L.ents[i];
    if (name) {
        strncpy(name, e.name.c_str(), 127);
        name[127] = 0;
    }
    if (shape) {
        shape[0] = e.shape[0];
        shape[1] = e.shape[1];
    }
    if (ndim) *ndim = e.ndim;
    if (offset) *offset = e.off;
    return 0;
}

int64_t slnlp_tf_arena_floats(const slnlp_tf_config* cfg) {
    if (check_cfg(cfg)) return -1;
    return build_layout(*cfg).total;
}

int64_t slnlp_tf_workspace_bytes(const slnlp_tf_config* cfg) {
    if (check_cfg(cfg)) return -1;
    return (int64_t)carve(*cfg, nullptr).bytes;
}

void slnlp_tf_destroy(slnlp_tf_plan* plan) {
    if (!plan) return;
    if (!plan->graphs.empty()) (void)hipDeviceSynchronize();
    else destroy_sync(plan->destroy_sync);
    for (auto& kv : plan->graphs) (void)hipGraphExecDestroy(kv.second);
    delete plan;
}

int slnlp_tf_create(const slnlp_tf_config* cfg, const slnlp_tf_buffers* buf, slnlp_tf_plan** out) {
    SLNLP_TRY(check_cfg(cfg));
    SLNLP_CHECK_ARG(buf && out, "tf_create: null argument");
    SLNLP_CHECK_ARG(buf->params && buf->grads && buf->momentum && buf->pe && buf->workspace && buf->rng && buf->lr &&
                        buf->scalars,
                    "tf_create: every buffer pointer is required");
    SLNLP_CHECK_ARG((((uintptr_t)buf->params | (uintptr_t)buf->grads | (uintptr_t)buf->momentum |
                      (uintptr_t)buf->workspace | (uintptr_t)buf->pe) & 255) == 0,
                    "tf_create: arenas / workspace / pe must be 256-byte aligned");
    slnlp_tf_plan* p = new slnlp_tf_plan();
    p->cfg = *cfg;
    p->buf = *buf;
    p->L = build_layout(*cfg);
    p->w = carve(*cfg, buf->workspace);
    bool ok = attn_init() == 0 && gemm_planes_init() == 0;
    p->use_planes = (cfg->E % 64 == 0) && (cfg->F % 64 == 0);
    p->wgrad_np = wgrad_passes();
    p->dgrad_np = dgrad_passes();
    {
        const char* e = getenv("SLNLP_DEC_ROWS");
        p->use_rows = p->use_planes && cfg->E <= 1024 && cfg->F <= 1024 && !(e && atoi(e) == 0);
    }
    if (ok && cfg->precision == 8) {
        std::vector<QuantRow> rows;
        auto block = [&](long off, int nrows, int K) {
            p->qrow0[off] = (long)rows.size();
            for (int r = 0; r < nrows; ++r) rows.push_back(QuantRow{off + (long)r * K, K, 0});
        };
        const int E = cfg->E, F = cfg->F;
        for (int i = 0; i < cfg->N; ++i) {
            const EncP& q = p->L.enc[i];
            block(q.in_w, 3 * E, E); block(q.out_w, E, E); block(q.l1_w, F, E); block(q.l2_w, E, F);
        }
        ok = (long)rows.size() == p->w.n_qrows &&
             hipMemcpy(p->w.qrow_table, rows.data(), rows.size() * sizeof(QuantRow), hipMemcpyHostToDevice) == hipSuccess;
    }
    std::vector<slnlp_ln_reduce_entry> tab;
    std::vector<LnPartialEntry> ptab;
    const int nbE = p->nbE = ln_bwd_blocks(cfg->B * cfg->S), nbD = p->nbD = ln_bwd_blocks(cfg->B);
    auto ent = [&](float* part, long gw, long gb, int dec, const float* dy, const float* x, const float* stats) {
        slnlp_ln_reduce_entry e;
        e.partial = part; e.dgamma = p->G(gw); e.dbeta = p->G(gb); e.nblk = dec ? nbD : nbE; e.E = cfg->E;
        tab.push_back(e);
        LnPartialEntry q;
        q.dy = dy; q.x = x; q.stats = stats; q.partial = part; q.dec = dec; q.pad = 0;
        ptab.push_back(q);
    };
    {
        const Ws& w = p->w;
        const int N = cfg->N;
        for (int i = 0; i < N; ++i) {
            const EncA& a = w.enc[i];
            ent(a.lnp1, p->L.enc[i].n1_w, p->L.enc[i].n1_b, 0, a.gx1, a.y1, a.st1);
            ent(a.lnp2, p->L.enc[i].n2_w, p->L.enc[i].n2_b, 0, i + 1 < N ? w.enc[i + 1].gx0 : w.gxl, a.y2, a.st2);
        }
        ent(w.lnp_mem, p->L.encn_w, p->L.encn_b, 0, w.gmem, w.enc[N - 1].x2, w.st_mem);
        for (int i = 0; i < N; ++i) {
            const DecA& a = w.dec[i];
            ent(a.lnp1, p->L.dec[i].n1_w, p->L.dec[i].n1_b, 1, a.gt1, a.y1, a.st1);
            ent(a.lnp2, p->L.dec[i].n2_w, p->L.dec[i].n2_b, 1, a.gt2, a.y2, a.st2);
            ent(a.lnp3, p->L.dec[i].n3_w, p->L.dec[i].n3_b, 1, i + 1 < N ? w.dec[i + 1].gt0 : w.gtl, a.y3, a.st3);
        }
        ent(w.lnp_fin, p->L.decn_w, p->L.decn_b, 1, w.gfin, w.dec[N - 1].t3, w.st_fin);
    }
    ok = ok && hipMemcpy(p->w.ln_table, tab.data(), tab.size() * sizeof(tab[0]), hipMemcpyHostToDevice) == hipSuccess &&
         hipMemcpy(p->w.ln_ptable, ptab.data(), ptab.size() * sizeof(ptab[0]), hipMemcpyHostToDevice) == hipSuccess &&
         hipMemset(buf->grads, 0, p->L.total * sizeof(float)) == hipSuccess &&
         hipStreamSynchronize(nullptr) == hipSuccess;
    if (!ok) {
        set_error("tf_create: device initialisation failed: %s", hipGetErrorString(hipGetLastError()));
        slnlp_tf_destroy(p);
        return SLNLP_ERR_LAUNCH;
    }
    *out = p;
    return 0;
}

}

int slnlp_tf_plan::dec_self_block(int l, const float* t, const PP* tp, int B, float p, hipStream_t st) const {
    const slnlp_tf_plan* pl = this;
    const int E = cfg.E, dh = E / cfg.H;
    const DecP& q = L.dec[l];
    const DecA& a = w.dec[l];
    if (use_rows) {
        SLNLP_TRY(pl->linear_r(*tp, B, E, q.sin_w + 2L * E * E, E, pl->P(q.sin_b) + 2 * E, a.v, E, 0, p, pl->dec_site(l, 0), nullptr, &a.vp, st, dh));
        SLNLP_TRY(pl->linear_r(a.vp, B, E, q.sout_w, E, pl->P(q.sout_b), a.y1, E, 0, p, pl->dec_site(l, 1), t, nullptr, st));
        SLNLP_TRY(layernorm_fwd(a.y1, pl->P(q.n1_w), pl->P(q.n1_b), B, E, 1e-5f, a.t1, a.st1, st, a.t1p.out()));
        SLNLP_TRY(pl->linear_r(a.t1p, B, E, q.cin_w, E, pl->P(q.cin_b), a.q, E, 0, 0.f, 0, nullptr, nullptr, st));
        return 0;
    }
    SLNLP_TRY(pl->linear(t, B, E, pl->P(q.sin_w) + 2L * E * E, E, pl->P(q.sin_b) + 2 * E, a.v, E, 0, p, pl->dec_site(l, 0), nullptr, st, dh));
    SLNLP_TRY(pl->linear(a.v, B, E, pl->P(q.sout_w), E, pl->P(q.sout_b), a.y1, E, 0, p, pl->dec_site(l, 1), t, st));
    SLNLP_TRY(layernorm_fwd(a.y1, pl->P(q.n1_w), pl->P(q.n1_b), B, E, 1e-5f, a.t1, a.st1, st));
    SLNLP_TRY(pl->linear(a.t1, B, E, pl->P(q.cin_w), E, pl->P(q.cin_b), a.q, E, 0, 0.f, 0, nullptr, st));
    return 0;
}

int slnlp_tf_plan::forward_impl(const int64_t* X, const int64_t* y, int B, int train, float* logp_out, hipStream_t st) {
    slnlp_tf_plan* pl = this;
    const slnlp_tf_config& c = pl->cfg;
    const int E = c.E, F = c.F, H = c.H, S = c.S, dh = E / H, M = S * B, Vp = (int)align_up(c.Vt, 4);
    const float p = train ? c.dropout : 0.f;
    const unsigned long long* rng = pl->buf.rng;
    pl->last_B = B; pl->last_p = p; pl->last_X = X; pl->last_y = y;

    const bool up = use_planes;
    if (up) {
        SLNLP_TRY(prepare_planes(B, st));
        SLNLP_TRY(ensure_wplanes(st));
        SLNLP_TRY(ensure_wq(st));
    }
    SLNLP_TRY(embed_fwd(y, 1, B, 1, E, c.Vt, pl->P(L.tgt_emb), pl->buf.pe, w.t0, sqrtf((float)E), p, SITE_TGT_EMB, rng, c.pad_tgt, st,
                        use_rows ? w.t0p.out() : PlaneOut{}));
    SLNLP_TRY(dec_self_block(0, w.t0, &w.t0p, B, p, st));
    SLNLP_TRY(embed_fwd(X, S, B, S, E, c.Vs, pl->P(L.src_emb), pl->buf.pe, w.x0, sqrtf((float)E), p, SITE_SRC_EMB, rng, -1, st,
                        up ? w.x0p.out() : PlaneOut{}, w.emb_keep));

    const float* x = w.x0;
    const PP* xp = &w.x0p;
    for (int l = 0; l < c.N; ++l) {
        const EncP& q = L.enc[l];
        const EncA& a = w.enc[l];
        if (up) {
            SLNLP_TRY(pl->linear_p(*xp, M, E, q.in_w, 3 * E, pl->P(q.in_b), a.qkv, 3 * E, 0, 0.f, 0, nullptr, nullptr, st));
            SLNLP_TRY(attn_self_fwd(a.qkv, X, S, c.pad_src, 1, B, S, H, dh, S <= 64 ? nullptr : a.ctx, a.probs, p, pl->enc_site(l, 0), rng, st, a.ctxp.out()));
            SLNLP_TRY(pl->linear_p(a.ctxp, M, E, q.out_w, E, pl->P(q.out_b), a.y1, E, 0, p, pl->enc_site(l, 1), x, nullptr, st));
            SLNLP_TRY(layernorm_fwd(a.y1, pl->P(q.n1_w), pl->P(q.n1_b), M, E, 1e-5f, a.x1, a.st1, st, a.x1p.out()));
            SLNLP_TRY(pl->linear_p(a.x1p, M, E, q.l1_w, F, pl->P(q.l1_b), a.h, F, 1, p, pl->enc_site(l, 2), nullptr, &a.hp, st));
            SLNLP_TRY(pl->linear_p(a.hp, M, F, q.l2_w, E, pl->P(q.l2_b), a.y2, E, 0, p, pl->enc_site(l, 3), a.x1, nullptr, st));
            SLNLP_TRY(layernorm_fwd(a.y2, pl->P(q.n2_w), pl->P(q.n2_b), M, E, 1e-5f, a.x2, a.st2, st, a.x2p.out()));
        } else {
            SLNLP_TRY(pl->linear(x, M, E, pl->P(q.in_w), 3 * E, pl->P(q.in_b), a.qkv, 3 * E, 0, 0.f, 0, nullptr, st));
            SLNLP_TRY(attn_self_fwd(a.qkv, X, S, c.pad_src, 1, B, S, H, dh, a.ctx, a.probs, p, pl->enc_site(l, 0), rng, st));
            SLNLP_TRY(pl->linear(a.ctx, M, E, pl->P(q.out_w), E, pl->P(q.out_b), a.y1, E, 0, p, pl->enc_site(l, 1), x, st));
            SLNLP_TRY(layernorm_fwd(a.y1, pl->P(q.n1_w), pl->P(q.n1_b), M, E, 1e-5f, a.x1, a.st1, st));
            SLNLP_TRY(pl->linear(a.x1, M, E, pl->P(q.l1_w), F, pl->P(q.l1_b), a.h, F, 1, p, pl->enc_site(l, 2), nullptr, st));
            SLNLP_TRY(pl->linear(a.h, M, F, pl->P(q.l2_w), E, pl->P(q.l2_b), a.y2, E, 0, p, pl->enc_site(l, 3), a.x1, st));
            SLNLP_TRY(layernorm_fwd(a.y2, pl->P(q.n2_w), pl->P(q.n2_b), M, E, 1e-5f, a.x2, a.st2, st));
        }
        x = a.x2;
        xp = &a.x2p;
    }
    SLNLP_TRY(layernorm_fwd(x, pl->P(L.encn_w), pl->P(L.encn_b), M, E, 1e-5f, w.mem, w.st_mem, st, up ? w.memp.out() : PlaneOut{}));

    const float* t = w.t0;
    const PP* tp = &w.t0p;
    for (int l = 0; l < c.N; ++l) {
        const DecP& q = L.dec[l];
        const DecA& a = w.dec[l];
        if (l > 0) SLNLP_TRY(dec_self_block(l, t, tp, B, p, st));
        {
            const float *Wk = pl->P(q.cin_w) + (long)E * E, *Wv = pl->P(q.cin_w) + 2L * E * E;
            const slnlp_gemm_args j1 = pl->head_expand(a.q, Wk, a.qk, B, H, dh);
            SLNLP_TRY(gemm_group(&j1, 1, st));
            SLNLP_TRY(xmem_fwd(a.qk, w.mem, pl->P(q.cin_b) + 2 * E, B, S, H, dh, a.mbar, a.psum, a.xprobs, a.xctx, p, pl->dec_site(l, 2), rng, st));
            slnlp_gemm_args j2 = pl->head_reduce(a.mbar, Wv, a.xctx, a.xctx, B, H, dh);
            if (use_rows) { j2.C_hi = a.xctxp.hi; j2.C_lo = a.xctxp.lo; j2.ldc_p = E; }
            SLNLP_TRY(gemm_group(&j2, 1, st));
        }
        if (use_rows) {
            SLNLP_TRY(pl->linear_r(a.xctxp, B, E, q.cout_w, E, pl->P(q.cout_b), a.y2, E, 0, p, pl->dec_site(l, 3), a.t1, nullptr, st));
            SLNLP_TRY(layernorm_fwd(a.y2, pl->P(q.n2_w), pl->P(q.n2_b), B, E, 1e-5f, a.t2, a.st2, st, a.t2p.out()));
            SLNLP_TRY(pl->linear_r(a.t2p, B, E, q.l1_w, F, pl->P(q.l1_b), a.h, F, 1, p, pl->dec_site(l, 4), nullptr, &a.hp, st));
            SLNLP_TRY(pl->linear_r(a.hp, B, F, q.l2_w, E, pl->P(q.l2_b), a.y3, E, 0, p, pl->dec_site(l, 5), a.t2, nullptr, st));
            SLNLP_TRY(layernorm_fwd(a.y3, pl->P(q.n3_w), pl->P(q.n3_b), B, E, 1e-5f, a.t3, a.st3, st, a.t3p.out()));
        } else {
            SLNLP_TRY(pl->linear(a.xctx, B, E, pl->P(q.cout_w), E, pl->P(q.cout_b), a.y2, E, 0, p, pl->dec_site(l, 3), a.t1, st));
            SLNLP_TRY(layernorm_fwd(a.y2, pl->P(q.n2_w), pl->P(q.n2_b), B, E, 1e-5f, a.t2, a.st2, st));
            SLNLP_TRY(pl->linear(a.t2, B, E, pl->P(q.l1_w), F, pl->P(q.l1_b), a.h, F, 1, p, pl->dec_site(l, 4), nullptr, st));
            SLNLP_TRY(pl->linear(a.h, B, F, pl->P(q.l2_w), E, pl->P(q.l2_b), a.y3, E, 0, p, pl->dec_site(l, 5), a.t2, st));
            SLNLP_TRY(layernorm_fwd(a.y3, pl->P(q.n3_w), pl->P(q.n3_b), B, E, 1e-5f, a.t3, a.st3, st));
        }
        t = a.t3;
        tp = &a.t3p;
    }
    if (use_rows) {
        SLNLP_TRY(layernorm_fwd(t, pl->P(L.decn_w), pl->P(L.decn_b), B, E, 1e-5f, w.tfin, w.st_fin, st, w.tfinp.out()));
        SLNLP_TRY(pl->linear_r(w.tfinp, B, E, L.lin_w, c.Vt, pl->P(L.lin_b), w.logits, Vp, 0, 0.f, 0, nullptr, nullptr, st));
    } else {
        SLNLP_TRY(layernorm_fwd(t, pl->P(L.decn_w), pl->P(L.decn_b), B, E, 1e-5f, w.tfin, w.st_fin, st));
        SLNLP_TRY(pl->linear(w.tfin, B, E, pl->P(L.lin_w), c.Vt, pl->P(L.lin_b), w.logits, Vp, 0, 0.f, 0, nullptr, st));
    }
    SLNLP_TRY(lsm_nll(w.logits, Vp, y, B, c.Vt, c.pad_tgt, w.logp, pl->buf.scalars, train ? w.dlogits : nullptr, Vp,
                      w.row_nll, st, nullptr, logp_out ? logp_out : ls_logp, logp_out ? nullptr : ls_dyn,
                      logp_out ? nullptr : ls_loss, (!logp_out && ls_dyn) ? ls_dyn + 1 : nullptr, pl->opts.loss()));
    return 0;
}

extern "C" {

int slnlp_tf_forward(slnlp_tf_plan* pl, const int64_t* X, const int64_t* y, int B, int train, float* logp_out,
                     void* stream) {
    SLNLP_CHECK_ARG(pl && X && y, "tf_forward: `X` and `y` are required parameters");
    SLNLP_CHECK_ARG(B > 0 && B <= pl->cfg.B, "tf_forward: batch %d outside 1..%d", B, pl->cfg.B);
    StepScope scope((hipStream_t)stream);
    SLNLP_TRY(scope.rc);
    return pl->forward_impl(X, y, B, train, logp_out, (hipStream_t)stream);
}

int slnlp_tf_seed_dlogp(slnlp_tf_plan* pl, const float* dlogp, void* stream) {
    SLNLP_CHECK_ARG(pl && dlogp && pl->last_B > 0, "tf_seed_dlogp: needs a prior forward");
    return lsm_bwd(pl->w.logp, dlogp, pl->last_B, pl->cfg.Vt, pl->w.dlogits, align_up(pl->cfg.Vt, 4), (hipStream_t)stream);
}

int slnlp_tf_backward(slnlp_tf_plan* pl, void* stream) {
    SLNLP_CHECK_ARG(pl && pl->last_B > 0, "tf_backward: needs a prior forward(train)");
    hipStream_t st = (hipStream_t)stream;
    StepScope scope(st);
    SLNLP_TRY(scope.rc);
    const slnlp_tf_config& c = pl->cfg;
    const Ws& w = pl->w;
    const Layout& L = pl->L;
    const int B = pl->last_B, E = c.E, F = c.F, H = c.H, S = c.S, dh = E / H, M = S * B, Vp = (int)align_up(c.Vt, 4);
    const float p = pl->last_p, ik = 1.f / (1.f - p);
    const unsigned long long* rng = pl->buf.rng;
    const int64_t *X = pl->last_X, *y = pl->last_y;
    const bool up = pl->use_planes;

    SLNLP_TRY(pl->wd_group_f(pl->wgrad_args(w.dlogits, Vp, B, c.Vt, w.tfin, E, pl->G(L.lin_w), pl->G(L.lin_b)),
                             pl->dgrad_args(w.dlogits, Vp, B, c.Vt, pl->P(L.lin_w), E, w.gfin, nullptr, 0.f, nullptr), st));
    SLNLP_TRY(layernorm_bwd(w.gfin, w.dec[c.N - 1].t3, pl->P(L.decn_w), w.st_fin, B, E, nullptr, w.gtl, nullptr, 0.f, 0,
                            rng, nullptr, nullptr, 0, st));
    const float* dt = w.gtl;
    for (int l = c.N - 1; l >= 0; --l) {
        const DecP& q = L.dec[l];
        const DecA& a = w.dec[l];
        const float* t_in = l > 0 ? w.dec[l - 1].t3 : w.t0;
        if (pl->use_rows) {
            const PlaneOut none{};
            const PP& t_inp = l > 0 ? w.dec[l - 1].t3p : w.t0p;
            SLNLP_TRY(layernorm_bwd(dt, a.y3, pl->P(q.n3_w), a.st3, B, E, nullptr, a.gA3, nullptr, p, pl->dec_site(l, 5), rng, nullptr, nullptr, 0, st,
                                    p == 0.f ? a.d3p.out() : none, p > 0.f ? a.d3p.out() : none));
            SLNLP_TRY(pl->wd_rows(a.d3p, B, E, q.l2_w, F, nullptr, &a.ghp, a.h, ik, nullptr, a.hp, q.l2_w, q.l2_b, st));
            SLNLP_TRY(pl->wd_rows(a.ghp, B, F, q.l1_w, E, a.gt2, nullptr, nullptr, 0.f, a.gA3, a.t2p, q.l1_w, q.l1_b, st));
            SLNLP_TRY(layernorm_bwd(a.gt2, a.y2, pl->P(q.n2_w), a.st2, B, E, nullptr, a.gA2, nullptr, p, pl->dec_site(l, 3), rng, nullptr, nullptr, 0, st,
                                    p == 0.f ? a.d2p.out() : none, p > 0.f ? a.d2p.out() : none));
            SLNLP_TRY(pl->wd_rows(a.d2p, B, E, q.cout_w, E, a.gxctx, nullptr, nullptr, 0.f, nullptr, a.xctxp, q.cout_w, q.cout_b, st));
            {
                const float *Wk = pl->P(q.cin_w) + (long)E * E, *Wv = pl->P(q.cin_w) + 2L * E * E;
                const slnlp_gemm_args j1 = pl->head_expand(a.gxctx, Wv, a.dmbar, B, H, dh);
                SLNLP_TRY(gemm_group(&j1, 1, st));
                SLNLP_TRY(xmem_bwd(w.mem, pl->P(q.cin_b) + 2 * E, a.xprobs, a.psum, a.qk, a.dmbar, a.gxctx, B, S, H, dh, a.dsc, a.dqk, a.dcp,
                                   pl->G(q.cin_b) + 2 * E, w.gmem, l == c.N - 1 ? 0 : 1, p, pl->dec_site(l, 2), rng, st));
                slnlp_gemm_args jobs[3] = {pl->head_reduce(a.dqk, Wk, a.gq, nullptr, B, H, dh),
                                           pl->head_wgrad(a.q, a.dqk, pl->G(q.cin_w) + (long)E * E, B, H, dh),
                                           pl->head_wgrad(a.gxctx, a.mbar, pl->G(q.cin_w) + 2L * E * E, B, H, dh)};
                jobs[0].C_hi = a.gqp.hi; jobs[0].C_lo = a.gqp.lo; jobs[0].ldc_p = E;
                SLNLP_TRY(gemm_group(jobs, 3, st));
            }
            SLNLP_TRY(pl->wd_rows(a.gqp, B, E, q.cin_w, E, a.gt1, nullptr, nullptr, 0.f, a.gA2, a.t1p, q.cin_w, q.cin_b, st));
            SLNLP_TRY(layernorm_bwd(a.gt1, a.y1, pl->P(q.n1_w), a.st1, B, E, nullptr, a.gA1, nullptr, p, pl->dec_site(l, 1), rng, nullptr, nullptr, 0, st,
                                    p == 0.f ? a.d1p.out() : none, p > 0.f ? a.d1p.out() : none));
            SLNLP_TRY(pl->wd_rows(a.d1p, B, E, q.sout_w, E, nullptr, &a.gvp, nullptr, 0.f, nullptr, a.vp, q.sout_w, q.sout_b, st, p, pl->dec_site(l, 0), p > 0.f ? dh : 0));
            SLNLP_TRY(pl->wd_rows(a.gvp, B, E, q.sin_w + 2L * E * E, E, a.gt0, nullptr, nullptr, 0.f, a.gA1, t_inp, q.sin_w + 2L * E * E, q.sin_b + 2 * E, st));
            dt = a.gt0;
            continue;
        }
        SLNLP_TRY(layernorm_bwd(dt, a.y3, pl->P(q.n3_w), a.st3, B, E, nullptr, a.gA3, p > 0.f ? a.gB3 : nullptr, p,
                                pl->dec_site(l, 5), rng, nullptr, nullptr, 0, st));
        const float* d3 = p > 0.f ? a.gB3 : a.gA3;
        SLNLP_TRY(pl->wd_group_f(pl->wgrad_args(d3, E, B, E, a.h, F, pl->G(q.l2_w), pl->G(q.l2_b)),
                                 pl->dgrad_args(d3, E, B, E, pl->P(q.l2_w), F, a.gh, a.h, ik, nullptr), st));
        SLNLP_TRY(pl->wd_group_f(pl->wgrad_args(a.gh, F, B, F, a.t2, E, pl->G(q.l1_w), pl->G(q.l1_b)),
                                 pl->dgrad_args(a.gh, F, B, F, pl->P(q.l1_w), E, a.gt2, nullptr, 0.f, a.gA3), st));
        SLNLP_TRY(layernorm_bwd(a.gt2, a.y2, pl->P(q.n2_w), a.st2, B, E, nullptr, a.gA2, p > 0.f ? a.gB2 : nullptr, p,
                                pl->dec_site(l, 3), rng, nullptr, nullptr, 0, st));
        const float* d2 = p > 0.f ? a.gB2 : a.gA2;
        SLNLP_TRY(pl->wd_group_f(pl->wgrad_args(d2, E, B, E, a.xctx, E, pl->G(q.cout_w), pl->G(q.cout_b)),
                                 pl->dgrad_args(d2, E, B, E, pl->P(q.cout_w), E, a.gxctx, nullptr, 0.f, nullptr), st));
        {
            const float *Wk = pl->P(q.cin_w) + (long)E * E, *Wv = pl->P(q.cin_w) + 2L * E * E;
            const slnlp_gemm_args j1 = pl->head_expand(a.gxctx, Wv, a.dmbar, B, H, dh);
            SLNLP_TRY(gemm_group(&j1, 1, st));
            SLNLP_TRY(xmem_bwd(w.mem, pl->P(q.cin_b) + 2 * E, a.xprobs, a.psum, a.qk, a.dmbar, a.gxctx, B, S, H, dh, a.dsc, a.dqk, a.dcp,
                               pl->G(q.cin_b) + 2 * E, w.gmem, l == c.N - 1 ? 0 : 1, p, pl->dec_site(l, 2), rng, st));
            const slnlp_gemm_args jobs[3] = {pl->head_reduce(a.dqk, Wk, a.gq, nullptr, B, H, dh),
                                             pl->head_wgrad(a.q, a.dqk, pl->G(q.cin_w) + (long)E * E, B, H, dh),
                                             pl->head_wgrad(a.gxctx, a.mbar, pl->G(q.cin_w) + 2L * E * E, B, H, dh)};
            SLNLP_TRY(gemm_group(jobs, 3, st));
        }
        SLNLP_TRY(pl->wd_group_f(pl->wgrad_args(a.gq, E, B, E, a.t1, E, pl->G(q.cin_w), pl->G(q.cin_b)),
                                 pl->dgrad_args(a.gq, E, B, E, pl->P(q.cin_w), E, a.gt1, nullptr, 0.f, a.gA2), st));
        hipStream_t sb = st;
        SLNLP_TRY(layernorm_bwd(a.gt1, a.y1, pl->P(q.n1_w), a.st1, B, E, nullptr, a.gA1, p > 0.f ? a.gB1 : nullptr, p,
                                pl->dec_site(l, 1), rng, nullptr, nullptr, 0, sb));
        const float* d1 = p > 0.f ? a.gB1 : a.gA1;
        {
            slnlp_gemm_args dg = pl->dgrad_args(d1, E, B, E, pl->P(q.sout_w), E, a.gv, nullptr, 0.f, nullptr);
            if (p > 0.f) { dg.drop_p = p; dg.drop_site = pl->dec_site(l, 0); dg.rng = rng; dg.drop_head_dim = dh; }
            SLNLP_TRY(pl->wd_group_f(pl->wgrad_args(d1, E, B, E, a.v, E, pl->G(q.sout_w), pl->G(q.sout_b)), dg, sb));
        }
        SLNLP_TRY(pl->wd_group_f(pl->wgrad_args(a.gv, E, B, E, t_in, E, pl->G(q.sin_w) + 2L * E * E, pl->G(q.sin_b) + 2 * E),
                                 pl->dgrad_args(a.gv, E, B, E, pl->P(q.sin_w) + 2L * E * E, E, a.gt0, nullptr, 0.f, a.gA1), sb));
        dt = a.gt0;
    }
    SLNLP_TRY(embed_bwd(y, 1, B, 1, E, c.Vt, dt, pl->G(L.tgt_emb), sqrtf((float)E), -1, p, SITE_TGT_EMB, rng, w.emb_scratch_tgt, st));

    const int Mfull = c.B * c.S;
    const bool lnf = ln_bwd_fused(Mfull);
    SLNLP_TRY(layernorm_bwd(w.gmem, w.enc[c.N - 1].x2, pl->P(L.encn_w), w.st_mem, M, E, nullptr, w.gxl, nullptr, 0.f, 0,
                            rng, lnf ? w.lnp_mem : nullptr, nullptr, Mfull, st));
    const float* dx = w.gxl;
    for (int l = c.N - 1; l >= 0; --l) {
        const EncP& q = L.enc[l];
        const EncA& a = w.enc[l];
        const float* x_in = l > 0 ? w.enc[l - 1].x2 : w.x0;
        const PP& xp_in = l > 0 ? w.enc[l - 1].x2p : w.x0p;
        const PlaneOut none{};
        SLNLP_TRY(layernorm_bwd(dx, a.y2, pl->P(q.n2_w), a.st2, M, E, nullptr, a.gA2, (p > 0.f && !up) ? a.gB2 : nullptr, p,
                                pl->enc_site(l, 3), rng, lnf ? a.lnp2 : nullptr, nullptr, Mfull, st, (up && p == 0.f) ? a.d2p.out() : none,
                                (up && p > 0.f) ? a.d2p.out() : none));
        const float* d2 = p > 0.f ? a.gB2 : a.gA2;
        if (up) {
            SLNLP_TRY(pl->wd_group(pl->wgrad_p_args(a.d2p, E, M, E, a.hp, F, pl->G(q.l2_w), pl->G(q.l2_b)),
                                   pl->dgrad_p_args(a.d2p, E, M, E, q.l2_w, F, nullptr, a.h, ik, nullptr, &a.ghp), 0, st));
            SLNLP_TRY(pl->wd_group(pl->wgrad_p_args(a.ghp, F, M, F, a.x1p, E, pl->G(q.l1_w), pl->G(q.l1_b)),
                                   pl->dgrad_p_args(a.ghp, F, M, F, q.l1_w, E, a.gx1, nullptr, 0.f, a.gA2, nullptr), 0, st));
        } else {
            SLNLP_TRY(pl->wd_group_f(pl->wgrad_args(d2, E, M, E, a.h, F, pl->G(q.l2_w), pl->G(q.l2_b)),
                                     pl->dgrad_args(d2, E, M, E, pl->P(q.l2_w), F, a.gh, a.h, ik, nullptr), st));
            SLNLP_TRY(pl->wd_group_f(pl->wgrad_args(a.gh, F, M, F, a.x1, E, pl->G(q.l1_w), pl->G(q.l1_b)),
                                     pl->dgrad_args(a.gh, F, M, F, pl->P(q.l1_w), E, a.gx1, nullptr, 0.f, a.gA2), st));
        }
        SLNLP_TRY(layernorm_bwd(a.gx1, a.y1, pl->P(q.n1_w), a.st1, M, E, nullptr, a.gA1, (p > 0.f && !up) ? a.gB1 : nullptr, p,
                                pl->enc_site(l, 1), rng, lnf ? a.lnp1 : nullptr, nullptr, Mfull, st, (up && p == 0.f) ? a.d1p.out() : none,
                                (up && p > 0.f) ? a.d1p.out() : none));
        const float* d1 = p > 0.f ? a.gB1 : a.gA1;
        if (up) {
            SLNLP_TRY(pl->wd_group(pl->wgrad_p_args(a.d1p, E, M, E, a.ctxp, E, pl->G(q.out_w), pl->G(q.out_b)),
                                   pl->dgrad_p_args(a.d1p, E, M, E, q.out_w, E, a.gctx, nullptr, 0.f, nullptr, nullptr), 0, st));
            SLNLP_TRY(attn_self_bwd(a.qkv, a.probs, a.gctx, B, S, H, dh, S <= 64 ? nullptr : a.gqkv, p, pl->enc_site(l, 0), rng, st, a.gqkvp.out(), w.attn_scratch));
// ... 207 lines not shown
```

### sign-language-nlp_amd/csrc/tf_plan.hpp

```cpp
#pragma once
#include <map>
#include <string>
#include <vector>

#include "common.hpp"
#include "launch.hpp"

namespace slnlp {

static inline long align_up(long v, long a) { return (v + a - 1) / a * a; }

struct ParamEnt {
    std::string name;
    int64_t shape[2];
    int ndim;
    int64_t off, numel;
};
struct EncP { long in_w, in_b, out_w, out_b, l1_w, l1_b, l2_w, l2_b, n1_w, n1_b, n2_w, n2_b; };
struct DecP {
    long sin_w, sin_b, sout_w, sout_b, cin_w, cin_b, cout_w, cout_b, l1_w, l1_b, l2_w, l2_b;
    long n1_w, n1_b, n2_w, n2_b, n3_w, n3_b;
};
struct Layout {
    std::vector<ParamEnt> ents;
// ... 196 lines not shown
        a.qk = b.take<float>(B * H * E);
        a.mbar = b.take<float>(B * H * E);
        a.psum = b.take<float>(B * H);
        a.xprobs = b.take<float>(B * H * S);
        a.xctx = b.take<float>(B * E);
        a.y2 = b.take<float>(B * E);
        a.st2 = b.take<float>(B * 2);
        a.t2 = b.take<float>(B * E);
        a.h = b.take<float>(B * F);
        a.y3 = b.take<float>(B * E);
        a.st3 = b.take<float>(B * 2);
        a.t3 = b.take<float>(B * E);
        a.lnp1 = b.take<float>(lnpD);
        a.lnp2 = b.take<float>(lnpD);
        a.lnp3 = b.take<float>(lnpD);
        a.gA3 = b.take<float>(B * E);
        a.gB3 = b.take<float>(B * E);
        a.gh = b.take<float>(B * F);
        a.gt2 = b.take<float>(B * E);
        a.gA2 = b.take<float>(B * E);
        a.gB2 = b.take<float>(B * E);
        a.gxctx = b.take<float>(B * E);
        a.gq = b.take<float>(B * E);
        a.dmbar = b.take<float>(B * H * E);
        a.dsc = b.take<float>(B * H * S);
        a.dqk = b.take<float>(B * H * E);
        a.dcp = b.take<float>(B * E);
        a.gt1 = b.take<float>(B * E);
        a.gA1 = b.take<float>(B * E);
        a.gB1 = b.take<float>(B * E);
        a.gv = b.take<float>(B * E);
        a.gt0 = b.take<float>(B * E);
        w.dec.push_back(a);
    }
    w.tfin = b.take<float>(B * E);
    w.st_fin = b.take<float>(B * 2);
    w.lnp_fin = b.take<float>(lnpD);
    w.logits = b.take<float>(B * Vp);
    w.dlogits = b.take<float>(B * Vp);
    w.logp = b.take<float>(B * c.Vt);
    w.row_nll = b.take<float>(B);
    w.gfin = b.take<float>(B * E);
    w.gtl = b.take<float>(B * E);
    w.gmem = b.take<float>(M * E);
    w.gxl = b.take<float>(M * E);
    w.emb_scratch_src = b.take<char>(embed_bwd_scratch_bytes(c.B, c.S, c.E));
    w.emb_scratch_tgt = b.take<char>(embed_bwd_scratch_bytes(c.B, 1, c.E));
    w.emb_keep = b.take<unsigned char>(M * E / 4);
    w.opt_partials = b.take<float>(1024);
    w.attn_scratch = c.S > 64 ? (float*)b.take<char>(attn_long_scratch_bytes(c.B, c.S, c.H)) : nullptr;
    w.ln_table = b.take<slnlp_ln_reduce_entry>(5 * c.N + 2);
    w.ln_ptable = b.take<LnPartialEntry>(5 * c.N + 2);
    const size_t Mp = (M + 63) / 64 * 64;
    const bool q8 = c.precision == 8;
    auto pp = [&](size_t cols, bool fwd_operand = false) {
        PP q;
        q.hi = b.take<unsigned short>(Mp * cols);
        q.lo = b.take<unsigned short>(Mp * cols);
        if (q8 && fwd_operand) q.q8 = b.take<unsigned char>(Mp * cols);
        return q;
    };
    const size_t wtot = (size_t)build_layout(c).total + 64 * 3 * (E > F ? E : F);
    w.wp.hi = b.take<unsigned short>(wtot);
    w.wp.lo = b.take<unsigned short>(wtot);
    w.n_qrows = (long)c.N * (3 * E + E + F + E);
    w.wq = q8 ? b.take<unsigned char>(wtot) : nullptr;
    w.wscale = q8 ? b.take<float>(w.n_qrows) : nullptr;
    w.qrow_table = q8 ? b.take<QuantRow>(w.n_qrows) : nullptr;
    b.cur = (b.cur + 255) & ~(size_t)255;
    w.planes_begin = b.base + b.cur;
    w.x0p = pp(E, true);
    w.memp = pp(E, true);
    for (int i = 0; i < c.N; ++i) {
        EncA& a = w.enc[i];
        a.ctxp = pp(E, true); a.x1p = pp(E, true); a.hp = pp(F, true); a.x2p = pp(E, true);
        a.d2p = pp(E); a.ghp = pp(F); a.d1p = pp(E); a.gqkvp = pp(3 * E);
    }
    {
        const size_t Bp = (B + 63) / 64 * 64;
        auto ppd = [&](size_t cols) {
            PP q;
            q.hi = b.take<unsigned short>(Bp * cols);
            q.lo = b.take<unsigned short>(Bp * cols);
            return q;
        };
        w.t0p = ppd(E);
        w.tfinp = ppd(E);
        for (int i = 0; i < c.N; ++i) {
            DecA& a = w.dec[i];
            a.vp = ppd(E); a.t1p = ppd(E); a.xctxp = ppd(E); a.t2p = ppd(E); a.hp = ppd(F); a.t3p = ppd(E);
            a.d3p = ppd(E); a.ghp = ppd(F); a.d2p = ppd(E); a.gqp = ppd(E); a.d1p = ppd(E); a.gvp = ppd(E);
        }
    }
    {
        const size_t nx = ((E > F ? E : F) + 255) / 256 * 256, ny = ((3 * E > F ? 3 * E : F) + 255) / 256 * 256;
        w.gscr_bytes = 16384 + nx * ny * MAX_SPLITK * sizeof(float) + ny * MAX_SPLITK * sizeof(float);
        w.gscr_bytes = (w.gscr_bytes + 255) & ~(size_t)255;
        w.gscr[0] = b.take<char>(w.gscr_bytes);
    }
    b.cur = (b.cur + 255) & ~(size_t)255;
    w.planes_end = b.base + b.cur;
    w.bytes = (b.cur + 255) & ~(size_t)255;
    return w;
}

}

using namespace slnlp;

enum { SITE_SRC_EMB = 1, SITE_TGT_EMB = 2, SITE_LAYER0 = 16, SITE_PER_LAYER = 8 };

struct slnlp_tf_plan {
    slnlp_tf_config cfg;
    slnlp_tf_buffers buf;
    Layout L;
    Ws w;
    int last_B = 0;
    float last_p = 0.f;
    const int64_t* last_X = nullptr;
    const int64_t* last_y = nullptr;
    std::map<int, hipGraphExec_t> graphs;
    TrainOpts opts;
    int nbE = 0, nbD = 0;
    int destroy_sync = 1;
    float* ls_logp = nullptr;
    float* ls_loss = nullptr;
    const int* ls_dyn = nullptr;
    int prec3() const { return cfg.precision == 8 ? 3 : cfg.precision; }
    unsigned long long wq_gen = 0;
    std::map<long, long> qrow0;
    int ensure_wq(hipStream_t st) {
        if (cfg.precision != 8) return 0;
        unsigned long long g = params_generation(buf.params);
        if (g != 0 && g == wq_gen) return 0;
        SLNLP_TRY(quant_rows_fp8(buf.params, 0, (int)w.n_qrows, 0, w.wq, 0, w.wscale, w.qrow_table, st));
        if (g == 0) g = bump_params_generation(buf.params);
        wq_gen = g;
        return 0;
    }
    unsigned long long wplanes_gen = 0;
    int ensure_wplanes(hipStream_t st) {
        if (!use_planes) return 0;
        unsigned long long g = params_generation(buf.params);
        if (g != 0 && g == wplanes_gen) return 0;
        SLNLP_TRY(split_planes(buf.params, L.total, 1, (int)L.total, w.wp.hi, w.wp.lo, L.total, st));
        if (g == 0) g = bump_params_generation(buf.params);
        wplanes_gen = g;
        return 0;
    }
    long wplane_begin() const { return L.enc.empty() ? 0 : L.enc[0].in_w; }
    long wplane_end() const { return L.enc.empty() ? 0 : (use_rows && cfg.B <= ROWS_MAX_B ? L.encn_w : L.total); }
    static constexpr int ROWS_MAX_B = 64;
    bool rows_for(int B, int drop_head_dim) const { return B <= ROWS_MAX_B || drop_head_dim != 0; }
    void params_stepped() {
        const unsigned long long g = bump_params_generation(buf.params);
        if (use_planes) wplanes_gen = g;
    }
    bool use_planes = false;
    bool use_rows = false;
    int wgrad_np = 2, dgrad_np = 2;
    int planes_B = -1;

    float* P(long off) const { return buf.params + off; }
    float* G(long off) const { return buf.grads + off; }
    int enc_site(int l, int k) const { return SITE_LAYER0 + l * SITE_PER_LAYER + k; }
    int dec_site(int l, int k) const { return SITE_LAYER0 + (cfg.N + l) * SITE_PER_LAYER + k; }

    int dec_self_block(int l, const float* t, const PP* tp, int B, float p, hipStream_t st) const;

    int linear(const float* x, int M, int K, const float* W, int N, const float* bias, float* y, long ldy, int relu,
               float p, int site, const float* resid, hipStream_t st, int drop_head_dim = 0) const {
        slnlp_gemm_args a;
        memset(&a, 0, sizeof(a));
        a.A = x; a.lda = K; a.a_kmajor = 1;
        a.B = W; a.ldb = K; a.b_kmajor = 1;
        a.C = y; a.ldc = ldy; a.M = M; a.N = N; a.K = K;
        a.bias = bias; a.relu = relu;
        a.drop_p = p; a.drop_site = site; a.rng = buf.rng;
        a.resid = resid; a.ldr = ldy;
        a.precision = prec3();
        a.drop_head_dim = drop_head_dim;
        return gemm(a, st);
    }
    slnlp_gemm_args dgrad_args(const float* dy, long ldy, int M, int Nout, const float* W, int Kin, float* dx,
                               const float* gate, float gate_scale, const float* resid) const {
        slnlp_gemm_args a;
        memset(&a, 0, sizeof(a));
        a.A = dy; a.lda = ldy; a.a_kmajor = 1;
        a.B = W; a.ldb = Kin; a.b_kmajor = 0;
        a.C = dx; a.ldc = Kin; a.M = M; a.N = Kin; a.K = Nout;
        a.gate = gate; a.ldg = Kin; a.gate_scale = gate_scale;
        a.resid = resid; a.ldr = Kin;
        a.precision = prec3();
        return a;
    }
    int dgrad(const float* dy, long ldy, int M, int Nout, const float* W, int Kin, float* dx, const float* gate,
              float gate_scale, const float* resid, hipStream_t st) const {
        return gemm(dgrad_args(dy, ldy, M, Nout, W, Kin, dx, gate, gate_scale, resid), st);
    }
    slnlp_gemm_args wgrad_args(const float* dy, long ldy, int T, int Nout, const float* x, int Kin, float* dW, float* db) const {
        slnlp_gemm_args a;
        memset(&a, 0, sizeof(a));
        a.A = dy; a.lda = ldy; a.a_kmajor = 0;
        a.B = x; a.ldb = Kin; a.b_kmajor = 0;
        a.C = dW; a.ldc = Kin; a.M = Nout; a.N = Kin; a.K = T;
        a.rowsum_a = db;
        a.precision = prec3();
        return a;
    }
    int wgrad(const float* dy, long ldy, int T, int Nout, const float* x, int Kin, float* dW, float* db,
              hipStream_t st) const {
        return gemm(wgrad_args(dy, ldy, T, Nout, x, Kin, dW, db), st);
    }
    static slnlp_gemm_args batched(slnlp_gemm_args a, int H, long sa, long sb, long sc) {
        a.batch = H; a.batch_stride_a = sa; a.batch_stride_b = sb; a.batch_stride_c = sc;
        return a;
    }
    slnlp_gemm_args head_expand(const float* x, const float* W, float* out, int B, int H, int dh) const {
        const int E = H * dh;
        slnlp_gemm_args a = dgrad_args(x, E, B, dh, W, E, out, nullptr, 0.f, nullptr);
        a.ldc = (long)H * E;
        return batched(a, H, dh, (long)dh * E, E);
    }
    slnlp_gemm_args head_reduce(const float* x, const float* W, float* out, const float* resid, int B, int H, int dh) const {
        const int E = H * dh;
        slnlp_gemm_args a;
        memset(&a, 0, sizeof(a));
        a.A = x; a.lda = (long)H * E; a.a_kmajor = 1;
        a.B = W; a.ldb = E; a.b_kmajor = 1;
        a.C = out; a.ldc = E; a.M = B; a.N = dh; a.K = E;
        a.resid = resid; a.ldr = E;
        a.precision = prec3();
        return batched(a, H, E, (long)dh * E, dh);
    }
    slnlp_gemm_args head_wgrad(const float* dy, const float* x, float* dW, int B, int H, int dh) const {
        const int E = H * dh;
        slnlp_gemm_args a = wgrad_args(dy, E, B, dh, x, E, dW, nullptr);
        a.ldb = (long)H * E;
        return batched(a, H, dh, E, (long)dh * E);
    }
    int wd_group_f(const slnlp_gemm_args& wg, const slnlp_gemm_args& dg, hipStream_t st) const {
        const slnlp_gemm_args jobs[2] = {wg, dg};
        return gemm_group(jobs, 2, st);
    }
    int linear_p(const PP& x, int M, int K, long woff, int N, const float* bias, float* y, long ldy, int relu, float p,
                 int site, const float* resid, const PP* outp, hipStream_t st) const {
        slnlp_gemm_args a;
        memset(&a, 0, sizeof(a));
        if (cfg.precision == 8) {
            a.A_hi = reinterpret_cast<const uint16_t*>(x.q8); a.lda_p = K; a.a_kmajor = 1;
            a.B_hi = reinterpret_cast<const uint16_t*>(w.wq + woff); a.ldb_p = K; a.b_kmajor = 1;
            a.col_scale = w.wscale + qrow0.at(woff);
            a.C = y; a.ldc = ldy; a.M = M; a.N = N; a.K = K;
            a.bias = bias; a.relu = relu;
            a.drop_p = p; a.drop_site = site; a.rng = buf.rng;
            a.resid = resid; a.ldr = ldy;
            if (outp) { a.C_hi = outp->hi; a.C_lo = outp->lo; a.C_q8 = outp->q8; a.ldc_p = N; }
            a.precision = 8;
            return gemm(a, st);
        }
        a.A_hi = x.hi; a.A_lo = x.lo; a.lda_p = K; a.a_kmajor = 1;
        a.B_hi = w.wp.hi + woff; a.B_lo = w.wp.lo + woff; a.ldb_p = K; a.b_kmajor = 1;
        a.C = y; a.ldc = ldy; a.M = M; a.N = N; a.K = K;
        a.bias = bias; a.relu = relu;
        a.drop_p = p; a.drop_site = site; a.rng = buf.rng;
        a.resid = resid; a.ldr = ldy;
        if (outp) { a.C_hi = outp->hi; a.C_lo = outp->lo; a.ldc_p = N; }
        a.precision = prec3();
        return gemm(a, st);
    }
    int linear_r(const PP& x, int M, int K, long woff, int N, const float* bias, float* y, long ldy, int relu, float p, int site,
                 const float* resid, const PP* outp, hipStream_t st, int drop_head_dim = 0) const {
        slnlp_gemm_args a;
        memset(&a, 0, sizeof(a));
        a.A_hi = x.hi; a.A_lo = x.lo; a.lda_p = K; a.a_kmajor = 1;
        const bool rows = rows_for(M, drop_head_dim);
        if (rows) { a.B = P(woff); a.ldb = K; }
        else { a.B_hi = w.wp.hi + woff; a.B_lo = w.wp.lo + woff; a.ldb_p = K; }
        a.b_kmajor = 1;
        a.C = y; a.ldc = ldy; a.M = M; a.N = N; a.K = K;
        a.bias = bias; a.relu = relu;
        a.drop_p = p; a.drop_site = site; a.rng = buf.rng;
        a.resid = resid; a.ldr = ldy;
        if (outp) { a.C_hi = outp->hi; a.C_lo = outp->lo; a.ldc_p = N; }
        a.precision = prec3();
        a.drop_head_dim = drop_head_dim;
        return rows ? gemm_rows(a, st) : gemm(a, st);
    }
    int wd_rows(const PP& dy, int B, int Nout, long woff, int Kin, float* dx, const PP* dxp, const float* gate, float gate_scale,
                const float* resid, const PP& x, long gw, long gb, hipStream_t st, float drop_p = 0.f, int drop_site = 0, int drop_head_dim = 0) const {
        if (!rows_for(B, drop_head_dim))
            return wd_group(wgrad_p_args(dy, Nout, B, Nout, x, Kin, G(gw), G(gb)),
                            dgrad_p_args(dy, Nout, B, Nout, woff, Kin, dx, gate, gate_scale, resid, dxp), 0, st);
        slnlp_gemm_args d, g;
        memset(&d, 0, sizeof(d));
        memset(&g, 0, sizeof(g));
        d.A_hi = dy.hi; d.A_lo = dy.lo; d.lda_p = Nout; d.a_kmajor = 1;
        d.B = P(woff); d.ldb = Kin; d.b_kmajor = 0;
        d.C = dx; d.ldc = Kin; d.M = B; d.N = Kin; d.K = Nout;
        d.gate = gate; d.ldg = Kin; d.gate_scale = gate_scale;
        d.resid = resid; d.ldr = Kin;
        if (dxp) { d.C_hi = dxp->hi; d.C_lo = dxp->lo; d.ldc_p = Kin; }
        d.drop_p = drop_p; d.drop_site = drop_site; d.rng = buf.rng; d.drop_head_dim = drop_head_dim;
        d.precision = prec3();
        g.A_hi = dy.hi; g.A_lo = dy.lo; g.lda_p = Nout; g.a_kmajor = 0;
        g.B_hi = x.hi; g.B_lo = x.lo; g.ldb_p = Kin; g.b_kmajor = 0;
        g.C = G(gw); g.ldc = Kin; g.M = Nout; g.N = Kin; g.K = B;
        g.rowsum_a = G(gb);
        g.precision = prec3();
        return gemm_rows_bwd(d, g, st);
    }
    slnlp_gemm_args dgrad_p_args(const PP& dy, long ldy, int M, int Nout, long woff, int Kin, float* dx, const float* gate,
                                 float gate_scale, const float* resid, const PP* outp) const {
        slnlp_gemm_args a;
        memset(&a, 0, sizeof(a));
        a.A_hi = dy.hi; a.A_lo = dy.lo; a.lda_p = ldy; a.a_kmajor = 1;
        a.B_hi = w.wp.hi + woff; a.B_lo = w.wp.lo + woff; a.ldb_p = Kin; a.b_kmajor = 0;
        a.C = dx; a.ldc = Kin; a.M = M; a.N = Kin; a.K = Nout;
        a.gate = gate; a.ldg = Kin; a.gate_scale = gate_scale;
        a.resid = resid; a.ldr = Kin;
        if (outp) { a.C_hi = outp->hi; a.C_lo = outp->lo; a.ldc_p = Kin; }
        a.precision = prec3() == 3 ? dgrad_np : prec3();
        return a;
    }
    int dgrad_p(const PP& dy, long ldy, int M, int Nout, long woff, int Kin, float* dx, const float* gate,
                float gate_scale, const float* resid, const PP* outp, hipStream_t st) const {
        return gemm(dgrad_p_args(dy, ldy, M, Nout, woff, Kin, dx, gate, gate_scale, resid, outp), st);
    }
    slnlp_gemm_args wgrad_p_args(const PP& dy, long ldy, int T, int Nout, const PP& x, int Kin, float* dW, float* db) const {
        slnlp_gemm_args a;
        memset(&a, 0, sizeof(a));
        a.A_hi = dy.hi; a.A_lo = dy.lo; a.lda_p = ldy; a.a_kmajor = 0;
        a.B_hi = x.hi; a.B_lo = x.lo; a.ldb_p = Kin; a.b_kmajor = 0;
        a.C = dW; a.ldc = Kin; a.M = Nout; a.N = Kin; a.K = T;
        a.rowsum_a = db;
        a.precision = prec3() == 3 ? wgrad_np : prec3();
        return a;
    }
    int wgrad_p(const PP& dy, long ldy, int T, int Nout, const PP& x, int Kin, float* dW, float* db, hipStream_t st) const {
        return gemm(wgrad_p_args(dy, ldy, T, Nout, x, Kin, dW, db), st);
    }
    int wd_group(const slnlp_gemm_args& wg, const slnlp_gemm_args& dg, int which_scratch, hipStream_t st) const {
        return gemm_planes_wd(wg, dg, w.gscr[which_scratch], w.gscr_bytes, st);
    }
    int prepare_planes(int B, hipStream_t st) {
        if (!use_planes || B == planes_B) return 0;
        if (hipMemsetAsync(w.planes_begin, 0, (size_t)(w.planes_end - w.planes_begin), st) != hipSuccess) {
            set_error("tf: zeroing operand planes failed");
            return SLNLP_ERR_LAUNCH;
        }
        planes_B = B;
        return 0;
    }
    int forward_impl(const int64_t* X, const int64_t* y, int B, int train, float* logp_out, hipStream_t st);
};
```

### sign-language-nlp_amd/slnlp/_lib.py

```python
import ctypes as C
import os

_HERE = os.path.dirname(os.path.abspath(__file__))
LIB_PATH = os.path.join(os.path.dirname(_HERE), "lib",
                        f"libslnlp_probe{os.environ['SLNLP_PROBE_LIB']}.so" if os.environ.get("SLNLP_PROBE_LIB") else "libslnlp.so")

i32, i64, f32, vp = C.c_int32, C.c_int64, C.c_float, C.c_void_p


class GemmArgs(C.Structure):
    _fields_ = [("A", vp), ("lda", i64), ("a_kmajor", i32),
                ("B", vp), ("ldb", i64), ("b_kmajor", i32),
                ("C", vp), ("ldc", i64),
                ("M", i32), ("N", i32), ("K", i32),
                ("bias", vp), ("relu", i32),
                ("gate", vp), ("ldg", i64), ("gate_scale", f32),
                ("drop_p", f32), ("drop_site", i32), ("rng", vp),
                ("resid", vp), ("ldr", i64),
                ("rowsum_a", vp), ("precision", i32), ("gate_mode", i32),
                ("A_hi", vp), ("A_lo", vp), ("lda_p", i64), ("B_hi", vp), ("B_lo", vp), ("ldb_p", i64),
                ("C_hi", vp), ("C_lo", vp), ("ldc_p", i64), ("drop_head_dim", i32),
                ("col_scale", vp), ("C_q8", vp),
                ("batch", i32), ("batch_stride_a", i64), ("batch_stride_b", i64), ("batch_stride_c", i64)]


class TimedLaunch(C.Structure):
    _fields_ = [("blocks", i32), ("njobs", i32), ("geometry", i32), ("us", f32)]


class TfConfig(C.Structure):
    _fields_ = [("E", i32), ("H", i32), ("N", i32), ("F", i32), ("Vs", i32), ("Vt", i32),
                ("B", i32), ("S", i32), ("pad_src", i32), ("pad_tgt", i32),
                ("dropout", f32), ("precision", i32)]


class TfBuffers(C.Structure):
    _fields_ = [("params", vp), ("grads", vp), ("momentum", vp), ("pe", vp), ("workspace", vp),
                ("rng", vp), ("lr", vp), ("scalars", vp)]


class RnnConfig(C.Structure):
    _fields_ = [("lstm", i32), ("E", i32), ("Hd", i32), ("N", i32), ("Vs", i32), ("Vt", i32), ("B", i32), ("S", i32),
                ("pad_src", i32), ("pad_tgt", i32), ("bos_idx", i32), ("dropout", f32), ("precision", i32)]


class RnnCellDir(C.Structure):
    _fields_ = [("xproj", vp), ("hproj", vp), ("h", vp), ("c", vp), ("hprev_save", vp), ("cprev_save", vp),
                ("acts", vp), ("hn_save", vp), ("out", vp), ("t", i32), ("out_row0", i32), ("out_col0", i32)]


class RnnStepDir(C.Structure):
    _fields_ = [("h_in", vp), ("h_out", vp), ("w_hh", vp), ("b_hh", vp), ("xproj", vp), ("c", vp), ("cprev_save", vp),
                ("acts", vp), ("hn_save", vp), ("out", vp), ("t", i32), ("out_row0", i32), ("out_col0", i32)]


class RnnLayerDir(C.Structure):
    _fields_ = [("hprev", vp), ("h_final", vp), ("w_hh", vp), ("b_hh", vp), ("xproj", vp), ("c", vp), ("cprev", vp),
                ("acts", vp), ("hn", vp), ("out", vp), ("out_col0", i32), ("reverse", i32)]


class RnnCellBwdDir(C.Structure):
    _fields_ = [("dh_state", vp), ("dc_state", vp), ("dout", vp), ("acts", vp), ("cprev_save", vp),
                ("hprev_save", vp), ("hn_save", vp), ("dgx", vp), ("dgh", vp), ("carry", vp),
                ("t", i32), ("out_row0", i32), ("out_col0", i32),
                ("dh_extra", vp), ("extra_stride", i64), ("n_extra", i32)]


class RnnStepBwdDir(C.Structure):
    _fields_ = [("cell", RnnCellBwdDir), ("dgh_next", vp), ("w_hh", vp)]


class LnReduceEntry(C.Structure):
    _fields_ = [("partial", vp), ("dgamma", vp), ("dbeta", vp), ("nblk", i32), ("E", i32)]


SIGNATURES = {
    "slnlp_last_error": (C.c_char_p, []),
    "slnlp_abi_version": (i32, []),
    "slnlp_gemm": (i32, [C.POINTER(GemmArgs), vp]),
    "slnlp_gemm_group_scratch_bytes": (i64, [C.POINTER(GemmArgs), C.POINTER(i32), i32]),
    "slnlp_set_rnn_step_tile": (i32, [i32]),
    "slnlp_gemm_group": (i32, [C.POINTER(GemmArgs), C.POINTER(i32), i32, vp, i64, vp]),
    "slnlp_gemm_wd": (i32, [C.POINTER(GemmArgs), C.POINTER(GemmArgs), vp, i64, vp]),
    "slnlp_gemm_wd_plan": (i32, [C.POINTER(GemmArgs), C.POINTER(GemmArgs), C.POINTER(i32), C.POINTER(i32), C.POINTER(i32), C.POINTER(i32)]),
    "slnlp_gemm_rows": (i32, [C.POINTER(GemmArgs), vp]),
    "slnlp_gemm_rows_bwd": (i32, [C.POINTER(GemmArgs), C.POINTER(GemmArgs), vp]),
    "slnlp_set_rows_tile": (i32, [i32]),
    "slnlp_quant_rows_fp8": (i32, [vp, i64, i32, i32, vp, i64, vp, vp]),
    "slnlp_split_planes": (i32, [vp, i64, i32, i32, vp, vp, i64, vp]),
    "slnlp_embed_fwd": (i32, [vp, i64, i32, i32, i32, i32, vp, vp, vp, f32, f32, i32, vp, i64, vp]),
    "slnlp_embed_bwd_scratch_bytes": (i64, [i32, i32, i32]),
    "slnlp_embed_bwd": (i32, [vp, i64, i32, i32, i32, i32, vp, vp, f32, i64, f32, i32, vp, vp, vp]),
    "slnlp_attn_self_fwd": (i32, [vp, vp, i64, i64, i32, i32, i32, i32, i32, vp, vp, f32, i32, vp, vp]),
    "slnlp_attn_self_bwd": (i32, [vp, vp, vp, i32, i32, i32, i32, vp, f32, i32, vp, vp]),
    "slnlp_attn_long_scratch_bytes": (i64, [i32, i32, i32]),
    "slnlp_attn_self_bwd_long": (i32, [vp, vp, vp, i32, i32, i32, i32, vp, vp, f32, i32, vp, vp]),
    "slnlp_attn_cross_fwd": (i32, [vp, vp, i64, i32, i32, i32, i32, vp, vp, f32, i32, vp, vp]),
    "slnlp_attn_cross_bwd": (i32, [vp, vp, i64, vp, vp, i32, i32, i32, i32, vp, vp, i64, f32, i32, vp, vp]),
    "slnlp_layernorm_fwd": (i32, [vp, vp, vp, i32, i32, f32, vp, vp, vp]),
    "slnlp_layernorm_bwd": (i32, [vp, vp, vp, vp, i32, i32, vp, vp, vp, f32, i32, vp, vp, C.POINTER(i32), vp]),
    "slnlp_ln_param_reduce": (i32, [vp, i32, i32, vp]),
    "slnlp_lsm_nll": (i32, [vp, i64, vp, i32, i32, i64, vp, vp, vp, i64, vp, vp]),
    "slnlp_lsm_nll_ex": (i32, [vp, i64, vp, i32, i32, i64, vp, f32, i32, vp, vp, vp, i64, vp, vp]),
    "slnlp_lsm_bwd": (i32, [vp, vp, i32, i32, vp, i64, vp]),
    "slnlp_clip_sgd_step": (i32, [vp, vp, vp, i64, vp, f32, f32, vp, vp, vp, vp]),
    "slnlp_clip_adam_step": (i32, [vp, vp, vp, vp, i64, vp, f32, f32, f32, f32, f32, vp, vp, vp, vp]),
    "slnlp_clip_sgd_step_ex": (i32, [vp, vp, vp, i64, vp, f32, f32, f32, i32, f32, vp, vp, vp, i64, i64, vp]),
    "slnlp_clip_adamw_step": (i32, [vp, vp, vp, vp, i64, vp, f32, f32, f32, f32, f32, vp, vp, vp, i64, i64, vp]),
    "slnlp_dropout_mask": (i32, [vp, i32, i32, f32, i32, vp, vp]),
    "slnlp_rnn_cell_fwd": (i32, [i32, C.POINTER(RnnCellDir), i32, i32, i32, vp, f32, i64, f32, i32, vp, vp]),
    "slnlp_rnn_layer_fwd": (i32, [i32, C.POINTER(RnnLayerDir), i32, i32, i32, i32, vp, f32, i64, f32, i32, vp, i32, vp,
                                  C.POINTER(i32), vp]),
    "slnlp_rnn_step_fwd": (i32, [i32, C.POINTER(RnnStepDir), i32, i32, i32, vp, f32, i64, f32, i32, vp, i32, vp]),
    "slnlp_rnn_cell_bwd": (i32, [i32, C.POINTER(RnnCellBwdDir), i32, i32, i32, vp, i64, f32, i32, vp, vp]),
    "slnlp_rnn_step_bwd": (i32, [i32, C.POINTER(RnnStepBwdDir), i32, i32, i32, vp, i64, f32, i32, vp, i32, vp]),
    "slnlp_bahdanau_fwd": (i32, [vp, vp, vp, vp, vp, i64, i64, i32, i32, i32, vp, vp, vp]),
    "slnlp_bahdanau_bwd": (i32, [vp, vp, vp, vp, vp, vp, i32, i32, i32, vp, vp, vp, vp, vp, vp]),
    "slnlp_rnn_num_params": (i32, [C.POINTER(RnnConfig)]),
    "slnlp_rnn_param_info": (i32, [C.POINTER(RnnConfig), i32, C.c_char_p, C.POINTER(i64 * 2), C.POINTER(i32),
                                   C.POINTER(i64)]),
    "slnlp_rnn_arena_floats": (i64, [C.POINTER(RnnConfig)]),
    "slnlp_rnn_workspace_bytes": (i64, [C.POINTER(RnnConfig)]),
    "slnlp_rnn_create": (i32, [C.POINTER(RnnConfig), C.POINTER(TfBuffers), C.POINTER(vp)]),
    "slnlp_rnn_destroy": (None, [vp]),
    "slnlp_rnn_forward": (i32, [vp, vp, vp, vp, i32, i32, vp, vp]),
    "slnlp_rnn_seed_dlogp": (i32, [vp, vp, vp]),
    "slnlp_rnn_backward": (i32, [vp, vp]),
    "slnlp_rnn_optim": (i32, [vp, f32, f32, vp]),
    "slnlp_rnn_optim_adam": (i32, [vp, vp, f32, f32, f32, f32, f32, vp]),
    "slnlp_rnn_set_destroy_sync": (i32, [vp, i32]),
    "slnlp_rnn_set_criterion": (i32, [vp, vp, f32, i32, vp]),
    "slnlp_rnn_set_update": (i32, [vp, i32, f32, f32, i32]),
    "slnlp_rnn_train_step": (i32, [vp, vp, vp, vp, i32, f32, f32, vp, vp]),
    "slnlp_rnn_graph_capture_train": (i32, [vp, vp, vp, vp, i32, f32, f32, vp, vp]),
    "slnlp_rnn_graph_launch": (i32, [vp, i32, vp]),
    "slnlp_rnn_set_persistent": (i32, [vp, i32]),
    "slnlp_rnn_set_fused_backward": (i32, [vp, i32]),
    "slnlp_rnn_health": (i32, [vp, C.POINTER(i32)]),
    "slnlp_rnn_tap": (i32, [vp, C.c_char_p, vp, i64, C.POINTER(i64), vp]),
    "slnlp_tf_num_params": (i32, [C.POINTER(TfConfig)]),
    "slnlp_tf_param_info": (i32, [C.POINTER(TfConfig), i32, C.c_char_p, C.POINTER(i64 * 2), C.POINTER(i32),
                                  C.POINTER(i64)]),
    "slnlp_tf_arena_floats": (i64, [C.POINTER(TfConfig)]),
    "slnlp_tf_workspace_bytes": (i64, [C.POINTER(TfConfig)]),
    "slnlp_tf_create": (i32, [C.POINTER(TfConfig), C.POINTER(TfBuffers), C.POINTER(vp)]),
    "slnlp_tf_destroy": (None, [vp]),
    "slnlp_tf_forward": (i32, [vp, vp, vp, i32, i32, vp, vp]),
    "slnlp_tf_seed_dlogp": (i32, [vp, vp, vp]),
    "slnlp_tf_backward": (i32, [vp, vp]),
    "slnlp_tf_optim": (i32, [vp, f32, f32, vp]),
    "slnlp_tf_train_step": (i32, [vp, vp, vp, i32, f32, f32, vp, vp]),
    "slnlp_tf_graph_capture_train": (i32, [vp, vp, vp, i32, f32, f32, vp, vp]),
    "slnlp_tf_graph_launch": (i32, [vp, i32, vp]),
    "slnlp_tf_tap": (i32, [vp, C.c_char_p, vp, i64, C.POINTER(i64), vp]),
    "slnlp_tf_params_changed": (i32, [vp]),
    "slnlp_tf_optim_adam": (i32, [vp, vp, f32, f32, f32, f32, f32, vp]),
    "slnlp_tf_debug_layout": (i32, [vp, C.c_char_p, i64]),
    "slnlp_tf_set_destroy_sync": (i32, [vp, i32]),
    "slnlp_tf_set_criterion": (i32, [vp, vp, f32, i32, vp]),
    "slnlp_tf_set_update": (i32, [vp, i32, f32, f32, i32]),
    "slnlp_set_stream_policy": (i32, [i32]),
    "slnlp_set_thread_stream_policy": (i32, [i32]),
    "slnlp_set_backward_passes": (i32, [i32, i32]),
    "slnlp_get_backward_passes": (i32, [C.POINTER(i32), C.POINTER(i32)]),
    "slnlp_launch_timer_start": (i32, [i32]),
    "slnlp_launch_timer_stop": (i32, [C.POINTER(TimedLaunch), i32]),
    "slnlp_set_plane_tile": (i32, [i32]),
    "slnlp_set_gemm_ks": (i32, [i32]),
    "slnlp_set_fp8_tile": (i32, [i32]),
    "slnlp_tf_lockstep_workspace_bytes": (i64, [vp, i32]),
    "slnlp_tf_lockstep_create": (i32, [vp, i32, vp, i64, vp, vp]),
    "slnlp_tf_lockstep_destroy": (None, [vp]),
    "slnlp_tf_lockstep_set_data": (i32, [vp, i32, vp, vp, i64, vp, vp, vp]),
    "slnlp_tf_lockstep_step": (i32, [vp, i32, i64, i32, i32, i32, C.c_float, C.c_float, vp]),
    "slnlp_tf_lockstep_epoch": (i32, [vp, i32, i32, i32, C.c_float, C.c_float, vp]),
    "slnlp_tf_lockstep_num_launches": (i32, [vp, i32, i32, i32]),
    "slnlp_tf_lockstep_set_adam": (i32, [vp, vp, f32, f32, f32, f32]),
    "slnlp_tf_lockstep_set_destroy_sync": (i32, [vp, i32]),
    "slnlp_rnn_lockstep_workspace_bytes": (i64, [vp, i32]),
    "slnlp_rnn_lockstep_create": (i32, [vp, i32, vp, i64, vp, vp]),
    "slnlp_rnn_lockstep_destroy": (None, [vp]),
    "slnlp_rnn_lockstep_set_data": (i32, [vp, i32, vp, vp, vp, i64, vp, vp, vp]),
    "slnlp_rnn_lockstep_step": (i32, [vp, i32, i64, i32, i32, i32, C.c_float, C.c_float, vp]),
    "slnlp_rnn_lockstep_epoch": (i32, [vp, i32, i32, i32, C.c_float, C.c_float, vp]),
    "slnlp_rnn_lockstep_num_launches": (i32, [vp, i32, i32, i32]),
    "slnlp_rnn_lockstep_set_adam": (i32, [vp, vp, f32, f32, f32, f32]),
    "slnlp_rnn_lockstep_set_destroy_sync": (i32, [vp, i32]),
}

_lib = None


def load():
    global _lib
    if _lib is None:
        if not os.path.exists(LIB_PATH):
            raise RuntimeError(f"libslnlp.so not built at {LIB_PATH}: the HIP extension is the "
                               "only compute path (no CPU fallback)")
        lib = C.CDLL(LIB_PATH)
        for name, (res, args) in SIGNATURES.items():
            fn = getattr(lib, name)
            fn.restype, fn.argtypes = res, args
        _lib = lib
    return _lib


def check(rc, what=""):
    if rc != 0:
        msg = load().slnlp_last_error().decode(errors="replace")
        raise RuntimeError(f"libslnlp {what} failed (code {rc}): {msg}")


def require_gpu():
    import torch
    if not torch.cuda.is_available():
        raise RuntimeError("slnlp: no MI355X visible -- the HIP path is the only compute path "
                           "(there is deliberately no CPU fallback)")


REDUCTIONS = {"mean": 0, "sum": 1}
UPDATE_KINDS = {"sgd": 0, "adam": 1, "adamw": 2}


def ptr(t):
    return None if t is None else t.data_ptr()


def stream_ptr():
    import torch
    return torch.cuda.current_stream().cuda_stream
```

Measured before the change: 20460 seq/s.

## Fuse decoder LayerNorm forward into the following rows GEMM prologue

Adds a gemm_rows_ln kernel that computes LayerNorm for each 16-row tile in a prologue, keeps the normalized rows in LDS as the A operand, and lets the bx==0 blocks write the normalized output, planes and stats. The decoder forward now uses it for the n1, n2, n3 and final norms when the rows path is active, which removes separate layernorm_fwd launches and an activation round-trip through global memory. The cost is that every column block recomputes the LayerNorm for its rows and needs a larger LDS footprint, which may lower occupancy. It is disabled when recording lockstep programs.

```diff
diff --git a/include/slnlp.h b/include/slnlp.h
--- a/include/slnlp.h
+++ b/include/slnlp.h
@@ -52,6 +52,14 @@
 int slnlp_gemm_wd_plan(const slnlp_gemm_args* wgrad, const slnlp_gemm_args* dgrad, int32_t* split, int32_t* separate, int32_t* geo_wgrad,
                        int32_t* geo_dgrad);
 int slnlp_gemm_rows(const slnlp_gemm_args* args, void* stream);
+typedef struct slnlp_rows_ln {
+    const float* x; int64_t ldx;
+    const float* gamma; const float* beta; float eps;
+    float* y; int64_t ldy;
+    uint16_t* y_hi; uint16_t* y_lo; int64_t ldy_p;
+    float* stats;
+} slnlp_rows_ln;
+int slnlp_gemm_rows_ln(const slnlp_gemm_args* args, const slnlp_rows_ln* ln, void* stream);
 int slnlp_gemm_rows_bwd(const slnlp_gemm_args* dgrad, const slnlp_gemm_args* wgrad, void* stream);
 int slnlp_set_rows_tile(int tile);
 int slnlp_quant_rows_fp8(const float* x, int64_t ld, int R, int K, uint8_t* q, int64_t ldq, float* scale, void* stream);
diff --git a/sign-language-nlp_amd/csrc/common.hpp b/sign-language-nlp_amd/csrc/common.hpp
--- a/sign-language-nlp_amd/csrc/common.hpp
+++ b/sign-language-nlp_amd/csrc/common.hpp
@@ -200,6 +200,30 @@
     v = row16_sum(v);
     return (lane_bcast(v, 0) + lane_bcast(v, 16)) + (lane_bcast(v, 32) + lane_bcast(v, 48));
 }
+constexpr int LN_MAXU = 4;
+__device__ __forceinline__ void ln_row(float4 (&v)[LN_MAXU], const float4 (&g)[LN_MAXU], const float4 (&bt)[LN_MAXU], int E, float eps,
+                                       int lane, float& mean, float& rstd) {
+    float s = 0.f;
+#pragma unroll
+    for (int u = 0; u < LN_MAXU; ++u) s += v[u].x + v[u].y + v[u].z + v[u].w;
+    mean = wave_sum(s) / (float)E;
+    float q = 0.f;
+#pragma unroll
+    for (int u = 0; u < LN_MAXU; ++u) {
+        if (lane * 4 + u * 256 < E) {
+            const float a = v[u].x - mean, b = v[u].y - mean, cc = v[u].z - mean, d = v[u].w - mean;
+            q += a * a + b * b + cc * cc + d * d;
+        }
+    }
+    rstd = 1.f / sqrtf(wave_sum(q) / (float)E + eps);
+#pragma unroll
+    for (int u = 0; u < LN_MAXU; ++u) {
+        float4 o;
+        o.x = (v[u].x - mean) * rstd * g[u].x + bt[u].x; o.y = (v[u].y - mean) * rstd * g[u].y + bt[u].y;
+        o.z = (v[u].z - mean) * rstd * g[u].z + bt[u].z; o.w = (v[u].w - mean) * rstd * g[u].w + bt[u].w;
+        v[u] = o;
+    }
+}
 __device__ __forceinline__ float wave_max(float v) {
     v = row16_max(v);
     return fmaxf(fmaxf(lane_bcast(v, 0), lane_bcast(v, 16)), fmaxf(lane_bcast(v, 32), lane_bcast(v, 48)));
@@ -212,6 +236,7 @@
 int gemm_group(const slnlp_gemm_args* jobs, int njobs, hipStream_t s, unsigned wide_mask = 0);
 int gemm_planes(const slnlp_gemm_args& a, hipStream_t s);
 int gemm_rows(const slnlp_gemm_args& a, hipStream_t s);
+int gemm_rows_ln(const slnlp_gemm_args& a, const slnlp_rows_ln& ln, hipStream_t s);
 int gemm_rows_bwd(const slnlp_gemm_args& dgrad, const slnlp_gemm_args& wgrad, hipStream_t s);
 int gemm_planes_init();
 int gemm_planes_group(const slnlp_gemm_args* jobs, const int* split_k, int njobs, void* scratch, size_t scratch_bytes,
diff --git a/sign-language-nlp_amd/csrc/elementwise.hip b/sign-language-nlp_amd/csrc/elementwise.hip
--- a/sign-language-nlp_amd/csrc/elementwise.hip
+++ b/sign-language-nlp_amd/csrc/elementwise.hip
@@ -284,8 +284,6 @@
     return 0;
 }
 
-constexpr int LN_MAXU = 4;
-
 __device__ __forceinline__ void layernorm_fwd_body(const float* __restrict__ x,
                                                             const float* __restrict__ gamma,
                                                             const float* __restrict__ beta, int rows, int E,
@@ -304,28 +302,14 @@
         g[u] = in ? *reinterpret_cast<const float4*>(gamma + c) : make_float4(0.f, 0.f, 0.f, 0.f);
         bt[u] = in ? *reinterpret_cast<const float4*>(beta + c) : make_float4(0.f, 0.f, 0.f, 0.f);
     }
-    float s = 0.f;
-#pragma unroll
-    for (int u = 0; u < LN_MAXU; ++u) s += v[u].x + v[u].y + v[u].z + v[u].w;
-    const float mean = wave_sum(s) / (float)E;
-    float q = 0.f;
-#pragma unroll
-    for (int u = 0; u < LN_MAXU; ++u) {
-        if (lane * 4 + u * 256 < E) {
-            const float a = v[u].x - mean, b = v[u].y - mean, cc = v[u].z - mean, d = v[u].w - mean;
-            q += a * a + b * b + cc * cc + d * d;
-        }
-    }
-    const float rstd = 1.f / sqrtf(wave_sum(q) / (float)E + eps);
+    float mean, rstd;
+    ln_row(v, g, bt, E, eps, lane, mean, rstd);
 #pragma unroll
     for (int u = 0; u < LN_MAXU; ++u) {
         const int c = lane * 4 + u * 256;
         if (c < E) {
-            float4 o;
-            o.x = (v[u].x - mean) * rstd * g[u].x + bt[u].x; o.y = (v[u].y - mean) * rstd * g[u].y + bt[u].y;
-            o.z = (v[u].z - mean) * rstd * g[u].z + bt[u].z; o.w = (v[u].w - mean) * rstd * g[u].w + bt[u].w;
-            *reinterpret_cast<float4*>(y + (long)row * E + c) = o;
-            store_planes4(po, (long)row * E + c, o);
+            *reinterpret_cast<float4*>(y + (long)row * E + c) = v[u];
+            store_planes4(po, (long)row * E + c, v[u]);
         }
     }
     if (lane == 0 && stats) {
diff --git a/sign-language-nlp_amd/csrc/gemm_rows.hip b/sign-language-nlp_amd/csrc/gemm_rows.hip
--- a/sign-language-nlp_amd/csrc/gemm_rows.hip
+++ b/sign-language-nlp_amd/csrc/gemm_rows.hip
@@ -83,9 +83,53 @@
     for (int e = 0; e < 8; ++e) x[e] = p[e * 16];
 }
 
-template <int NSPLIT, int MT, int NT, bool BK>
-__device__ __forceinline__ void rows_tile(const RowsParams& p, int bx, int by, float* part) {
+constexpr int RT_LN_PAD = 4;
+__device__ __forceinline__ void rows_ln_prologue(const slnlp_rows_ln& q, int M, int K, int m0, bool store, float* img, int wave, int lane) {
+    const int ld = K + RT_LN_PAD;
+    float4 g[LN_MAXU], bt[LN_MAXU];
+#pragma unroll
+    for (int u = 0; u < LN_MAXU; ++u) {
+        const int c = lane * 4 + u * 256;
+        const bool in = c < K;
+        g[u] = in ? *reinterpret_cast<const float4*>(q.gamma + c) : make_float4(0.f, 0.f, 0.f, 0.f);
+        bt[u] = in ? *reinterpret_cast<const float4*>(q.beta + c) : make_float4(0.f, 0.f, 0.f, 0.f);
+    }
+    const PlaneOut po{q.y_hi, q.y_lo, nullptr};
+#pragma unroll
+    for (int r = wave; r < 16; r += RT_WAVES) {
+        const int row = m0 + r;
+        const float* xr = q.x + (long)min(row, M - 1) * q.ldx;
+        float4 v[LN_MAXU];
+#pragma unroll
+        for (int u = 0; u < LN_MAXU; ++u) {
+            const int c = lane * 4 + u * 256;
+            v[u] = c < K ? *reinterpret_cast<const float4*>(xr + c) : make_float4(0.f, 0.f, 0.f, 0.f);
+        }
+        float mean, rstd;
+        ln_row(v, g, bt, K, q.eps, lane, mean, rstd);
+        const bool out = store && row < M;
+#pragma unroll
+        for (int u = 0; u < LN_MAXU; ++u) {
+            const int c = lane * 4 + u * 256;
+            if (c < K) {
+                *reinterpret_cast<float4*>(img + r * ld + c) = v[u];
+                if (out) {
+                    if (q.y) *reinterpret_cast<float4*>(q.y + (long)row * q.ldy + c) = v[u];
+                    store_planes4(po, (long)row * q.ldy_p + c, v[u]);
+                }
+            }
+        }
+        if (out && lane == 0 && q.stats) {
+            q.stats[2 * row] = mean;
+            q.stats[2 * row + 1] = rstd;
+        }
+    }
+}
+
+template <int NSPLIT, int MT, int NT, bool BK, bool LN = false>
+__device__ __forceinline__ void rows_tile(const RowsParams& p, int bx, int by, float* part, const slnlp_rows_ln* ln = nullptr) {
     static_assert(MT * NT <= RT_WAVES, "one epilogue tile per wave");
+    static_assert(!LN || (MT == 1 && NT == 1 && BK), "the LayerNorm prologue: 16 x 16 forward tiles");
     const slnlp_gemm_args& g = p.a;
     const int tid = threadIdx.x, lane = tid & 63, wave = __builtin_amdgcn_readfirstlane(tid >> 6);
 #if SLNLP_PROBE_FENCES == 256
@@ -122,6 +166,11 @@
         bw[j] = g.B + (long)min(bcol[j] + (lane & 15), N - 1) * g.ldb + koct;
     }
     float* bimg = part + (size_t)ktiles * MT * NT * 256 + wave * NT * RT_FIMG;
+    float* lnimg = part + (size_t)ktiles * MT * NT * 256;
+    if constexpr (LN) {
+        rows_ln_prologue(*ln, M, g.K, bm0, bx == 0, lnimg, wave, lane);
+        __syncthreads();
+    }
 
     const int ei = wave / NT, ej = wave % NT;
     const int gm0 = bm0 + 16 * ei + ((lane >> 4) << 2), gn = bn0 + 16 * ej + (lane & 15);
@@ -157,6 +206,13 @@
                     rows_load8(bw[j] + k, x);
                     rows_split8<NSPLIT>(x, fb[kk][j], lb[kk][j]);
                 }
+            }
+            if constexpr (LN) {
+                const float* src = lnimg + (lane & 15) * (g.K + RT_LN_PAD) + k + koct;
+                const float4 x0 = *reinterpret_cast<const float4*>(src), x1 = *reinterpret_cast<const float4*>(src + 4);
+                const float x[8] = {x0.x, x0.y, x0.z, x0.w, x1.x, x1.y, x1.z, x1.w};
+                rows_split8<NSPLIT>(x, fa[kk][0], la[kk][0]);
+                continue;
             }
 #pragma unroll
             for (int i = 0; i < MT; ++i) {
@@ -384,6 +440,26 @@
 SLNLP_ROWS_KERNEL(1, 1)
 SLNLP_ROWS_KERNEL(1, 2)
 
+struct RowsLnParams {
+    RowsParams r;
+    slnlp_rows_ln ln;
+};
+__device__ __forceinline__ RowsLnParams as_global(RowsLnParams p) {
+    launder(p.r.a);
+    p.ln.x = as_global(p.ln.x); p.ln.gamma = as_global(p.ln.gamma); p.ln.beta = as_global(p.ln.beta);
+    p.ln.y = as_global(p.ln.y); p.ln.y_hi = as_global(p.ln.y_hi); p.ln.y_lo = as_global(p.ln.y_lo); p.ln.stats = as_global(p.ln.stats);
+    return p;
+}
+template <int NSPLIT>
+__device__ __forceinline__ void gemm_rows_ln_body(RowsLnParams p) {
+    extern __shared__ __attribute__((aligned(16))) float part[];
+    rows_tile<NSPLIT, 1, 1, true, true>(p.r, blockIdx.x, blockIdx.y, part, &p.ln);
+}
+__device__ __forceinline__ void gemm_rows_ln_body_3(RowsLnParams p) { gemm_rows_ln_body<3>(p); }
+__device__ __forceinline__ void gemm_rows_ln_body_1(RowsLnParams p) { gemm_rows_ln_body<1>(p); }
+SLNLP_ZKERNEL(gemm_rows_ln_kernel_3, RT_THREADS, gemm_rows_ln_body_3)
+SLNLP_ZKERNEL(gemm_rows_ln_kernel_1, RT_THREADS, gemm_rows_ln_body_1)
+
 using RowsKernel = void (*)(Pack<RowsParams>, const Pack<RowsParams>*);
 using RowsBwdKernel = void (*)(Pack<RowsBwdParams>, const Pack<RowsBwdParams>*);
 static RowsKernel rows_kernel(int precision, int geo) {
@@ -395,6 +471,7 @@
     return geo == 0 ? gemm_rows_bwd_kernel_1_0 : geo == 1 ? gemm_rows_bwd_kernel_1_1 : gemm_rows_bwd_kernel_1_2;
 }
 static size_t rows_lds(int geo, int K) { return (size_t)ceil_div(K, 64) * RT_GEO[geo].mt * RT_GEO[geo].nt * 64 * 4 * sizeof(float); }
+static size_t rows_ln_lds(int K) { return rows_lds(0, K) + (size_t)16 * (K + RT_LN_PAD) * sizeof(float); }
 static size_t rows_bwd_lds(int geo, int K) {
     const size_t d = rows_lds(geo, K) + (size_t)RT_WAVES * RT_GEO[geo].nt * RT_FIMG * sizeof(float);
     const size_t w = (size_t)(RT_GEO[geo].mt + RT_WAVES) * 2 * RT_IMG * sizeof(unsigned short);
@@ -432,6 +509,8 @@
                                                (int)std::min(rows_lds(geo, 64 * RT_MAX_KTILES), RT_LDS_MAX)) == hipSuccess &&
                      hipFuncSetAttribute((const void*)rows_bwd_kernel(prec, geo), hipFuncAttributeMaxDynamicSharedMemorySize,
                                          (int)std::min(rows_bwd_lds(geo, 64 * RT_MAX_KTILES), RT_LDS_MAX)) == hipSuccess;
+        for (const void* fn : {(const void*)gemm_rows_ln_kernel_3, (const void*)gemm_rows_ln_kernel_1})
+            ok = ok && hipFuncSetAttribute(fn, hipFuncAttributeMaxDynamicSharedMemorySize, (int)rows_ln_lds(64 * RT_MAX_KTILES)) == hipSuccess;
         if (!ok) {
             set_error("gemm_rows: cannot raise dynamic LDS limit: %s", hipGetErrorString(hipGetLastError()));
             return SLNLP_ERR_LAUNCH;
@@ -519,6 +598,25 @@
     return zlaunch(rows_kernel(a.precision, geo), rows_grid(geo, a.M, a.N), RT_THREADS, rows_lds(geo, a.K), st, "gemm_rows", p);
 }
 
+int gemm_rows_ln(const slnlp_gemm_args& a_in, const slnlp_rows_ln& ln, hipStream_t st) {
+    SLNLP_CHECK_ARG(!recording(), "gemm_rows_ln: not recordable (lockstep programs issue layernorm_fwd + gemm_rows)");
+    SLNLP_CHECK_ARG(ln.x && ln.gamma && ln.beta && a_in.K <= LN_MAXU * 256 && ln.ldx >= a_in.K && ln.ldx % 4 == 0 && (!ln.y_hi || ln.y_lo) &&
+                        (((uintptr_t)ln.x | (uintptr_t)ln.gamma | (uintptr_t)ln.beta | (uintptr_t)ln.y | (uintptr_t)ln.y_hi | (uintptr_t)ln.y_lo) & 15) == 0 &&
+                        (!ln.y || (ln.ldy >= a_in.K && ln.ldy % 4 == 0)) && (!ln.y_hi || (ln.ldy_p >= a_in.K && ln.ldy_p % 4 == 0)),
+                    "gemm_rows_ln: LayerNorm operand: K <= %d, 16-byte aligned rows, hi and lo planes together", LN_MAXU * 256);
+    slnlp_gemm_args a = a_in;
+    a.A_hi = reinterpret_cast<const uint16_t*>(ln.x); a.A_lo = a.A_hi; a.lda_p = (a.K + 63) / 64 * 64;
+    SLNLP_TRY(check_rows_job(a, true, "gemm_rows_ln"));
+    RowsLnParams p;
+    p.r.a = a;
+    p.r.drop_thr = dropout_threshold(a.drop_p);
+    p.r.drop_scale = 1.f / (1.f - a.drop_p);
+    p.ln = ln;
+    SLNLP_TRY(rows_init());
+    return zlaunch(a.precision == 3 ? gemm_rows_ln_kernel_3 : gemm_rows_ln_kernel_1, rows_grid(0, a.M, a.N), RT_THREADS, rows_ln_lds(a.K), st,
+                   "gemm_rows_ln", p);
+}
+
 }
 
 #if SLNLP_PROBE_FENCES == 256
@@ -559,3 +657,10 @@
     }
     return slnlp::gemm_rows(*args, (hipStream_t)stream);
 }
+extern "C" int slnlp_gemm_rows_ln(const slnlp_gemm_args* args, const slnlp_rows_ln* ln, void* stream) {
+    if (!args || !ln) {
+        slnlp::set_error("gemm_rows_ln: null args");
+        return SLNLP_ERR_INVALID_ARG;
+    }
+    return slnlp::gemm_rows_ln(*args, *ln, (hipStream_t)stream);
+}
diff --git a/sign-language-nlp_amd/csrc/tf_plan.hip b/sign-language-nlp_amd/csrc/tf_plan.hip
--- a/sign-language-nlp_amd/csrc/tf_plan.hip
+++ b/sign-language-nlp_amd/csrc/tf_plan.hip
@@ -130,14 +130,18 @@
 
 }
 
-int slnlp_tf_plan::dec_self_block(int l, const float* t, const PP* tp, int B, float p, hipStream_t st) const {
+int slnlp_tf_plan::dec_self_block(int l, const float* t, const PP* tp, int B, float p, hipStream_t st, const float* ln_in, long ln_w, long ln_b,
+                                  float* ln_out, float* ln_stats) const {
     const slnlp_tf_plan* pl = this;
     const int E = cfg.E, dh = E / cfg.H;
     const DecP& q = L.dec[l];
     const DecA& a = w.dec[l];
     if (use_rows) {
-        SLNLP_TRY(pl->linear_r(*tp, B, E, q.sin_w + 2L * E * E, E, pl->P(q.sin_b) + 2 * E, a.v, E, 0, p, pl->dec_site(l, 0), nullptr, &a.vp, st, dh));
+        SLNLP_TRY(pl->linear_r(*tp, B, E, q.sin_w + 2L * E * E, E, pl->P(q.sin_b) + 2 * E, a.v, E, 0, p, pl->dec_site(l, 0), nullptr, &a.vp, st, dh,
+                               ln_in, ln_w, ln_b, ln_out, ln_stats));
         SLNLP_TRY(pl->linear_r(a.vp, B, E, q.sout_w, E, pl->P(q.sout_b), a.y1, E, 0, p, pl->dec_site(l, 1), t, nullptr, st));
+        if (pl->ln_fused(B))
+            return pl->linear_r(a.t1p, B, E, q.cin_w, E, pl->P(q.cin_b), a.q, E, 0, 0.f, 0, nullptr, nullptr, st, 0, a.y1, q.n1_w, q.n1_b, a.t1, a.st1);
         SLNLP_TRY(layernorm_fwd(a.y1, pl->P(q.n1_w), pl->P(q.n1_b), B, E, 1e-5f, a.t1, a.st1, st, a.t1p.out()));
         SLNLP_TRY(pl->linear_r(a.t1p, B, E, q.cin_w, E, pl->P(q.cin_b), a.q, E, 0, 0.f, 0, nullptr, nullptr, st));
         return 0;
@@ -201,7 +205,11 @@
     for (int l = 0; l < c.N; ++l) {
         const DecP& q = L.dec[l];
         const DecA& a = w.dec[l];
-        if (l > 0) SLNLP_TRY(dec_self_block(l, t, tp, B, p, st));
+        if (l > 0) {
+            const DecA& b = w.dec[l - 1];
+            if (pl->ln_fused(B)) SLNLP_TRY(dec_self_block(l, t, tp, B, p, st, b.y3, L.dec[l - 1].n3_w, L.dec[l - 1].n3_b, b.t3, b.st3));
+            else SLNLP_TRY(dec_self_block(l, t, tp, B, p, st));
+        }
         {
             const float *Wk = pl->P(q.cin_w) + (long)E * E, *Wv = pl->P(q.cin_w) + 2L * E * E;
             const slnlp_gemm_args j1 = pl->head_expand(a.q, Wk, a.qk, B, H, dh);
@@ -212,11 +220,13 @@
             SLNLP_TRY(gemm_group(&j2, 1, st));
         }
         if (use_rows) {
+            const bool lnf = pl->ln_fused(B);
             SLNLP_TRY(pl->linear_r(a.xctxp, B, E, q.cout_w, E, pl->P(q.cout_b), a.y2, E, 0, p, pl->dec_site(l, 3), a.t1, nullptr, st));
-            SLNLP_TRY(layernorm_fwd(a.y2, pl->P(q.n2_w), pl->P(q.n2_b), B, E, 1e-5f, a.t2, a.st2, st, a.t2p.out()));
-            SLNLP_TRY(pl->linear_r(a.t2p, B, E, q.l1_w, F, pl->P(q.l1_b), a.h, F, 1, p, pl->dec_site(l, 4), nullptr, &a.hp, st));
+            if (!lnf) SLNLP_TRY(layernorm_fwd(a.y2, pl->P(q.n2_w), pl->P(q.n2_b), B, E, 1e-5f, a.t2, a.st2, st, a.t2p.out()));
+            SLNLP_TRY(pl->linear_r(a.t2p, B, E, q.l1_w, F, pl->P(q.l1_b), a.h, F, 1, p, pl->dec_site(l, 4), nullptr, &a.hp, st, 0,
+                                   lnf ? a.y2 : nullptr, q.n2_w, q.n2_b, a.t2, a.st2));
             SLNLP_TRY(pl->linear_r(a.hp, B, F, q.l2_w, E, pl->P(q.l2_b), a.y3, E, 0, p, pl->dec_site(l, 5), a.t2, nullptr, st));
-            SLNLP_TRY(layernorm_fwd(a.y3, pl->P(q.n3_w), pl->P(q.n3_b), B, E, 1e-5f, a.t3, a.st3, st, a.t3p.out()));
+            if (!lnf || l + 1 == c.N) SLNLP_TRY(layernorm_fwd(a.y3, pl->P(q.n3_w), pl->P(q.n3_b), B, E, 1e-5f, a.t3, a.st3, st, a.t3p.out()));
         } else {
             SLNLP_TRY(pl->linear(a.xctx, B, E, pl->P(q.cout_w), E, pl->P(q.cout_b), a.y2, E, 0, p, pl->dec_site(l, 3), a.t1, st));
             SLNLP_TRY(layernorm_fwd(a.y2, pl->P(q.n2_w), pl->P(q.n2_b), B, E, 1e-5f, a.t2, a.st2, st));
@@ -228,8 +238,10 @@
         tp = &a.t3p;
     }
     if (use_rows) {
-        SLNLP_TRY(layernorm_fwd(t, pl->P(L.decn_w), pl->P(L.decn_b), B, E, 1e-5f, w.tfin, w.st_fin, st, w.tfinp.out()));
-        SLNLP_TRY(pl->linear_r(w.tfinp, B, E, L.lin_w, c.Vt, pl->P(L.lin_b), w.logits, Vp, 0, 0.f, 0, nullptr, nullptr, st));
+        const bool lnf = pl->ln_fused(B);
+        if (!lnf) SLNLP_TRY(layernorm_fwd(t, pl->P(L.decn_w), pl->P(L.decn_b), B, E, 1e-5f, w.tfin, w.st_fin, st, w.tfinp.out()));
+        SLNLP_TRY(pl->linear_r(w.tfinp, B, E, L.lin_w, c.Vt, pl->P(L.lin_b), w.logits, Vp, 0, 0.f, 0, nullptr, nullptr, st, 0,
+                               lnf ? t : nullptr, L.decn_w, L.decn_b, w.tfin, w.st_fin));
     } else {
         SLNLP_TRY(layernorm_fwd(t, pl->P(L.decn_w), pl->P(L.decn_b), B, E, 1e-5f, w.tfin, w.st_fin, st));
         SLNLP_TRY(pl->linear(w.tfin, B, E, pl->P(L.lin_w), c.Vt, pl->P(L.lin_b), w.logits, Vp, 0, 0.f, 0, nullptr, st));
diff --git a/sign-language-nlp_amd/csrc/tf_plan.hpp b/sign-language-nlp_amd/csrc/tf_plan.hpp
--- a/sign-language-nlp_amd/csrc/tf_plan.hpp
+++ b/sign-language-nlp_amd/csrc/tf_plan.hpp
@@ -372,6 +372,7 @@
     long wplane_end() const { return L.enc.empty() ? 0 : (use_rows && cfg.B <= ROWS_MAX_B ? L.encn_w : L.total); }
     static constexpr int ROWS_MAX_B = 64;
     bool rows_for(int B, int drop_head_dim) const { return B <= ROWS_MAX_B || drop_head_dim != 0; }
+    bool ln_fused(int B) const { return use_rows && B <= ROWS_MAX_B && cfg.E <= 1024 && !recording(); }
     void params_stepped() {
         const unsigned long long g = bump_params_generation(buf.params);
         if (use_planes) wplanes_gen = g;
@@ -386,7 +387,8 @@
     int enc_site(int l, int k) const { return SITE_LAYER0 + l * SITE_PER_LAYER + k; }
     int dec_site(int l, int k) const { return SITE_LAYER0 + (cfg.N + l) * SITE_PER_LAYER + k; }
 
-    int dec_self_block(int l, const float* t, const PP* tp, int B, float p, hipStream_t st) const;
+    int dec_self_block(int l, const float* t, const PP* tp, int B, float p, hipStream_t st, const float* ln_in = nullptr, long ln_w = 0,
+                       long ln_b = 0, float* ln_out = nullptr, float* ln_stats = nullptr) const;
 
     int linear(const float* x, int M, int K, const float* W, int N, const float* bias, float* y, long ldy, int relu,
                float p, int site, const float* resid, hipStream_t st, int drop_head_dim = 0) const {
@@ -490,7 +492,8 @@
         return gemm(a, st);
     }
     int linear_r(const PP& x, int M, int K, long woff, int N, const float* bias, float* y, long ldy, int relu, float p, int site,
-                 const float* resid, const PP* outp, hipStream_t st, int drop_head_dim = 0) const {
+                 const float* resid, const PP* outp, hipStream_t st, int drop_head_dim = 0, const float* ln_in = nullptr, long ln_w = 0,
+                 long ln_b = 0, float* ln_out = nullptr, float* ln_stats = nullptr) const {
         slnlp_gemm_args a;
         memset(&a, 0, sizeof(a));
         a.A_hi = x.hi; a.A_lo = x.lo; a.lda_p = K; a.a_kmajor = 1;
@@ -505,6 +508,13 @@
         if (outp) { a.C_hi = outp->hi; a.C_lo = outp->lo; a.ldc_p = N; }
         a.precision = prec3();
         a.drop_head_dim = drop_head_dim;
+        if (ln_in) {
+            slnlp_rows_ln q;
+            memset(&q, 0, sizeof(q));
+            q.x = ln_in; q.ldx = K; q.gamma = P(ln_w); q.beta = P(ln_b); q.eps = 1e-5f;
+            q.y = ln_out; q.ldy = K; q.y_hi = x.hi; q.y_lo = x.lo; q.ldy_p = K; q.stats = ln_stats;
+            return gemm_rows_ln(a, q, st);
+        }
         return rows ? gemm_rows(a, st) : gemm(a, st);
     }
     int wd_rows(const PP& dy, int B, int Nout, long woff, int Kin, float* dx, const PP* dxp, const float* gate, float gate_scale,
diff --git a/sign-language-nlp_amd/slnlp/_lib.py b/sign-language-nlp_amd/slnlp/_lib.py
--- a/sign-language-nlp_amd/slnlp/_lib.py
+++ b/sign-language-nlp_amd/slnlp/_lib.py
@@ -70,6 +70,11 @@
     _fields_ = [("cell", RnnCellBwdDir), ("dgh_next", vp), ("w_hh", vp)]
 
 
+class RowsLn(C.Structure):
+    _fields_ = [("x", vp), ("ldx", i64), ("gamma", vp), ("beta", vp), ("eps", f32),
+                ("y", vp), ("ldy", i64), ("y_hi", vp), ("y_lo", vp), ("ldy_p", i64), ("stats", vp)]
+
+
 class LnReduceEntry(C.Structure):
     _fields_ = [("partial", vp), ("dgamma", vp), ("dbeta", vp), ("nblk", i32), ("E", i32)]
 
@@ -84,6 +89,7 @@
     "slnlp_gemm_wd": (i32, [C.POINTER(GemmArgs), C.POINTER(GemmArgs), vp, i64, vp]),
     "slnlp_gemm_wd_plan": (i32, [C.POINTER(GemmArgs), C.POINTER(GemmArgs), C.POINTER(i32), C.POINTER(i32), C.POINTER(i32), C.POINTER(i32)]),
     "slnlp_gemm_rows": (i32, [C.POINTER(GemmArgs), vp]),
+    "slnlp_gemm_rows_ln": (i32, [C.POINTER(GemmArgs), C.POINTER(RowsLn), vp]),
     "slnlp_gemm_rows_bwd": (i32, [C.POINTER(GemmArgs), C.POINTER(GemmArgs), vp]),
     "slnlp_set_rows_tile": (i32, [i32]),
     "slnlp_quant_rows_fp8": (i32, [vp, i64, i32, i32, vp, i64, vp, vp]),
```

After: 20670 seq/s, median of 6. +1.1%, better.
